# nka77/DAHiTra

Hardware: NVIDIA B200
Metric: image-pairs/sec (higher is better)
Workload: dtype x3 error-compensated f16 products (f16 main + scaled-remainder corrections; decoder: 3xTF32), fp32 accumulate

## Files before the change

### dahitra_b200/_lib.py

```python
from __future__ import annotations

import ctypes as C
import os
import subprocess
import threading

_HERE = os.path.dirname(os.path.abspath(__file__))
_CSRC = os.path.join(_HERE, "csrc")
LIB_PATH = os.path.join(_HERE, "libdahitra_b200.so")
SOURCES = ["conv_ffma.cu", "conv_tc.cu", "conv_tc2.cu", "conv_tc3.cu", "split.cu", "tokens.cu", "decoder.cu", "decoder_tc.cu", "stem_tc.cu", "classifier.cu", "train_decoder.cu", "train_tokens.cu", "prepare.cu", "aux.cu", "forward.cu"]
NVCC_FLAGS = ["-gencode", "arch=compute_100a,code=sm_100a", "-O3", "-lineinfo", "-std=c++17",
              "-Xcompiler", "-fPIC", "-shared"]

_lock = threading.Lock()
_lib = None


def _sources():
    return [os.path.join(_CSRC, s) for s in SOURCES if os.path.exists(os.path.join(_CSRC, s))]


STAMP_PATH = LIB_PATH + ".stamp"


def _deps():
    deps = _sources() + [os.path.join(_HERE, "..", "include", "dahitra_b200.h")]
    deps += [os.path.join(_CSRC, f) for f in sorted(os.listdir(_CSRC)) if f.endswith(".cuh")]
    return [d for d in deps if os.path.exists(d)]


def _source_hash() -> str:
    import hashlib
    h = hashlib.sha256(" ".join(NVCC_FLAGS + [os.environ.get("DAHITRA_DEBUG_BUILD", "0")]).encode())
    for d in _deps():
        h.update(os.path.basename(d).encode() + b"\0")
        with open(d, "rb") as f:
            h.update(f.read())
    return h.hexdigest()


def needs_build() -> bool:
    if not os.path.exists(LIB_PATH):
        return True
    if os.path.exists(STAMP_PATH):
        with open(STAMP_PATH) as f:
            return f.read().strip() != _source_hash()
    t = os.path.getmtime(LIB_PATH)
    if any(os.path.getmtime(d) > t for d in _deps()):
        return True
    _write_stamp()
    return False


def _write_stamp():
    try:
        with open(STAMP_PATH + ".tmp", "w") as f:
            f.write(_source_hash() + "\n")
        os.replace(STAMP_PATH + ".tmp", STAMP_PATH)
    except OSError:
        pass


def build(force: bool = False, verbose: bool = False) -> str:
    if not force and not needs_build():
        return LIB_PATH
    import tempfile
    from concurrent.futures import ThreadPoolExecutor
    nvcc = os.environ.get("NVCC", "nvcc")
    cflags = [f for f in NVCC_FLAGS if f != "-shared"]
    if os.environ.get("DAHITRA_DEBUG_BUILD") == "1":
        cflags.append("-DDH_MBAR_TIMEOUT")
    with tempfile.TemporaryDirectory(prefix="_build_", dir=_HERE) as tmp:
        def compile_one(src):
            obj = os.path.join(tmp, os.path.basename(src) + ".o")
            cmd = [nvcc] + cflags + ["-c", src, "-o", obj]
            if verbose:
                print(" ".join(cmd), flush=True)
            r = subprocess.run(cmd, capture_output=True, text=True)
            if r.returncode != 0:
                raise RuntimeError("nvcc failed on %s:\n%s%s" % (src, r.stdout, r.stderr))
            return obj
        with ThreadPoolExecutor(max_workers=min(8, os.cpu_count() or 1)) as ex:
            objs = list(ex.map(compile_one, _sources()))
        cmd = [nvcc] + NVCC_FLAGS + objs + ["-o", LIB_PATH + ".tmp"]
        if verbose:
            print(" ".join(cmd), flush=True)
        r = subprocess.run(cmd, capture_output=True, text=True)
        if r.returncode != 0:
            raise RuntimeError("nvcc link failed:\n" + r.stdout + r.stderr)
    os.replace(LIB_PATH + ".tmp", LIB_PATH)
    _write_stamp()
    return LIB_PATH


EXAMPLE_SRC = os.path.join(_HERE, "..", "examples", "dahitra_infer.c")
EXAMPLE_BIN = os.path.join(_HERE, "..", "examples", "bin", "dahitra_infer")


def build_example(force: bool = False, verbose: bool = False) -> str:
    src, out = os.path.abspath(EXAMPLE_SRC), os.path.abspath(EXAMPLE_BIN)
    deps = [src, LIB_PATH, os.path.join(_HERE, "..", "include", "dahitra_b200.h")]
    if not force and os.path.exists(out) and all(os.path.getmtime(d) <= os.path.getmtime(out) for d in deps):
        return out
    cuda = os.environ.get("CUDA_HOME", "/usr/local/cuda")
    os.makedirs(os.path.dirname(out), exist_ok=True)
    cmd = [os.environ.get("CC", "gcc"), "-std=c99", "-O2", "-Wall", "-Wextra", "-Werror", "-I", os.path.join(_HERE, "..", "include"),
           "-I", os.path.join(cuda, "include"), src, "-L", _HERE, "-ldahitra_b200", "-L", os.path.join(cuda, "lib64"),
           "-l:libcudart_static.a", "-ldl", "-lpthread", "-lrt", "-Wl,-rpath,$ORIGIN/../../dahitra_b200", "-o", out + ".tmp"]
    if verbose:
        print(" ".join(cmd), flush=True)
    r = subprocess.run(cmd, capture_output=True, text=True)
    if r.returncode != 0:
        raise RuntimeError("building examples/dahitra_infer.c failed:\n" + r.stdout + r.stderr)
    os.replace(out + ".tmp", out)
    return out


_P, _I, _LL, _SZ = C.c_void_p, C.c_int, C.c_longlong, C.c_size_t
SIGNATURES = {
    "dahitra_version": (_I, []),
    "dahitra_error_string": (C.c_char_p, [_I]),
    "dahitra_weight_slot_name": (C.c_char_p, [_I]),
    "dahitra_workspace_bytes": (_SZ, [_I, _I, _I, _I, _I, _I]),
    "dahitra_prepare_weights": (_LL, [_P, _I, _I, _I, _P, _LL, _P]),
    "dahitra_forward": (_I, [_P, _I, _P, _P, _LL, _P, _P, _P, _SZ, _I, _I, _I, _I, _I, _I, _P]),
    "dahitra_forward_profiled": (_I, [_P, _I, _P, _P, _LL, _P, _P, _P, _SZ, _I, _I, _I, _I, _I, _I, _P,
                                      _I, _P, _P, _P, _P]),
    "dahitra_conv2d": (_I, [_P, _P, _I, _I, _I, _I, _I, _I, _I, _I, _I, _I, _I, _P, _P, _P, _P, _I, _P, _I, _P]),
    "dahitra_conv2d_up2_tc": (_I, [_P, _I, _I, _I, _P, _P, _I, _P, _I, _P]),
    "dahitra_stem": (_I, [_P, _LL, _I, _I, _I, _P, _P, _P, _P]),
    "dahitra_stem_tc": (_I, [_P, _LL, _I, _I, _I, _P, _P, _P, _I, _P]),
    "dahitra_maxpool3x3s2": (_I, [_P, _I, _I, _I, _I, _P, _P]),
    "dahitra_squeeze_tokens": (_I, [_P, _I, _I, _I, _P, _P, _P, _P, _P]),
    "dahitra_token_encoder": (_I, [_P, _I, _I, _P, _I, _I, _P, _P]),
    "dahitra_decoder_tables": (_I, [_P, _I, _I, _I, _P, _I, _I, _P, _P]),
    "dahitra_pixel_decoder": (_I, [_P, _P, _P, _P, _I, _I, _I, _I, _I, _P, _I, _P, _P]),
    "dahitra_decoder_tables_tc": (_I, [_P, _I, _I, _I, _P, _I, _I, _P, _P]),
    "dahitra_pixel_decoder_tc": (_I, [_P, _P, _P, _P, _I, _I, _I, _I, _I, _P, _I, _I, _P, _P]),
    "dahitra_confusion_matrix": (_I, [_P, _P, _LL, _I, _P, _P]),
    "dahitra_prepare_input_u8": (_I, [_P, _I, _I, _I, _I, _I, _P, _P]),
    "dahitra_classifier": (_I, [_P, _I, _I, _I, _I, _P, _P, _P, _P, _P]),
    "dahitra_split_pack": (_I, [_P, _LL, _P, _P]),
    "dahitra_split_unpack": (_I, [_P, _LL, _P, _P]),
    "dahitra_maxpool3x3s2_split": (_I, [_P, _I, _I, _I, _I, _P, _P]),
    "dahitra_pixel_decoder_train_blocks": (_I, [_I]),
    "dahitra_pixel_decoder_train_fwd": (_I, [_P, _P, _P, _P, _I, _I, _I, _I, _I, _P]),
    "dahitra_pixel_decoder_train_bwd": (_I, [_P, _P, _P, _P, _P, _I, _I, _I, _I, _I, _P]),
    "dahitra_tokenizer_train_chunks": (_I, [_I]),
    "dahitra_tokenizer_train_fwd": (_I, [_P, _P, _P, _P, _P, _I, _I, _I, _P]),
    "dahitra_tokenizer_train_bwd": (_I, [_P, _P, _P, _P, _P, _P, _P, _I, _I, _I, _P]),
    "dahitra_conv2d_split": (_I, [_P, _P, _I, _I, _LL, _LL, _I, _I, _I, _I, _I, _I, _P, _P, _P, _I, _I, _P, _I, _I, _P, _P, _P]),
    "dahitra_maxpool3x3s2_h16": (_I, [_P, _I, _I, _I, _I, _P, _P]),
    "dahitra_classifier_h16": (_I, [_P, _I, _I, _I, _I, _P, _P, _P, _P, _P]),
}


class DhTensor(C.Structure):
    _fields_ = [("name", C.c_char_p), ("data", C.c_void_p), ("dtype", C.c_int), ("ndim", C.c_int), ("shape", C.c_longlong * 4)]


def load():
    global _lib
    with _lock:
        if _lib is None:
            if not os.path.exists(LIB_PATH):
                raise RuntimeError(
                    f"dahitra_b200: {LIB_PATH} is missing — run `python -c 'import __graft_entry__ as g; g.build()'` "
                    "(nvcc, sm_100a). There is no fallback path.")
            lib = C.CDLL(LIB_PATH)
            for name, (res, args) in SIGNATURES.items():
                fn = getattr(lib, name)
                fn.restype, fn.argtypes = res, args
            _lib = lib
        return _lib


def check(rc: int, what: str = "dahitra"):
    if rc != 0:
        msg = load().dahitra_error_string(rc)
        raise RuntimeError(f"{what} failed with code {rc}: {msg.decode() if msg else '?'}")
```

### dahitra_b200/csrc/common.cuh

```cuda
#pragma once
#include <cuda_runtime.h>
#include <stdint.h>
#include <stddef.h>
#include "../../include/dahitra_b200.h"

#ifndef __CUDA_ARCH_LIST__
#endif

#define DH_CHECK_LAUNCH()                                   \
  do {                                                      \
    cudaError_t e__ = cudaGetLastError();                   \
    if (e__ != cudaSuccess) return (int)e__;                \
  } while (0)

#define DH_REQUIRE(cond, code) \
  do {                         \
    if (!(cond)) return (code);\
  } while (0)

static inline bool dh_aligned16(const void* p) { return (reinterpret_cast<uintptr_t>(p) & 15u) == 0; }
static inline int dh_cdiv(int a, int b) { return (a + b - 1) / b; }

__device__ __forceinline__ float4 ldg4(const float* p) { return __ldg(reinterpret_cast<const float4*>(p)); }
__device__ __forceinline__ void st4(float* p, float4 v) { *reinterpret_cast<float4*>(p) = v; }

__device__ __forceinline__ float warp_sum(float v) {
#pragma unroll
  for (int o = 16; o > 0; o >>= 1) v += __shfl_xor_sync(0xffffffffu, v, o);
  return v;
}
__device__ __forceinline__ float warp_max(float v) {
#pragma unroll
  for (int o = 16; o > 0; o >>= 1) v = fmaxf(v, __shfl_xor_sync(0xffffffffu, v, o));
  return v;
}

__device__ __forceinline__ float gelu_erf(float x) { return 0.5f * x * (1.0f + erff(x * 0.70710678118654752440f)); }

struct ConvArgs {
  const float* in0; const float* in1; int C0, C1;
  int N, inH, inW, up;
  int KH, KW, stride, pad, Cout;
  const float* w;
  const float* wt;
  const float* bias; const float* res; int relu;
  float* out;
  int ps = 0;
  int flat = 0;
};
struct Conv3Args {
  const void* in0; const void* in1; int C0, C1;
  int N, inH, inW;
  long long in0_plane = 0, in1_plane = 0;
  long long res_plane = 0, out_plane = 0;
  int K, stride, Cout;
  const void* wt16;
  long long wt_plane_bytes;
  const float* bias; const void* res; int res_split;
  int relu;
  void* out; int out_split;
  int ps = 0;
  int tok = 0;
  const float* wtok = nullptr; float* partials = nullptr;
  int force_stream = 0;
  int cg = 0;
  int h16 = 0;
};
bool dh_conv_tc3_eligible(const Conv3Args& a);
int dh_launch_conv_tc3(const Conv3Args& a, cudaStream_t s);
int dh_conv_tc3_tok_chunks(int H, int W);
int dh_launch_split_pack(const float* in, size_t n, void* out, cudaStream_t s);
int dh_launch_split_unpack(const void* in, size_t n, float* out, cudaStream_t s);
int dh_launch_maxpool_split(const void* in, int N, int H, int W, int C, void* out, cudaStream_t s);
int dh_launch_maxpool_h16(const void* in, int N, int H, int W, int C, void* out, cudaStream_t s);
int dh_pdl_attr(cudaLaunchAttribute* at);
void dh_set_pdl(int on);
template <typename... KArgs, typename... Args>
static inline int dh_launch(void (*kern)(KArgs...), dim3 grid, dim3 block, size_t smem, cudaStream_t s, Args... args) {
  cudaLaunchConfig_t cfg = {};
  cfg.gridDim = grid; cfg.blockDim = block; cfg.dynamicSmemBytes = smem; cfg.stream = s;
  cudaLaunchAttribute at[1];
  cfg.attrs = at; cfg.numAttrs = dh_pdl_attr(at);
  const cudaError_t e = cudaLaunchKernelEx(&cfg, kern, KArgs(args)...);
  if (e != cudaSuccess) return (int)e;
  DH_CHECK_LAUNCH();
  return 0;
}
#ifdef __CUDACC__
__device__ __forceinline__ void dh_pdl_wait() { asm volatile("griddepcontrol.wait;" ::: "memory"); }
__device__ __forceinline__ void dh_pdl_launch_dependents() { asm volatile("griddepcontrol.launch_dependents;" ::: "memory"); }
#endif
int dh_launch_conv_ffma(const ConvArgs& a, cudaStream_t s);
bool dh_conv_tc_eligible(const ConvArgs& a);
int dh_launch_conv_tc(const ConvArgs& a, cudaStream_t s);
bool dh_conv_tc2_eligible(const ConvArgs& a);
int dh_launch_conv_tc2(const ConvArgs& a, int xm, int cg, cudaStream_t s);
int dh_launch_stem(const float* x, long long xbs, int N, int H, int W, const float* w, const float* b, float* out, cudaStream_t s);
int dh_launch_stem_tc(const float* x, long long xbs, int N, int H, int W, const float* wtc, const float* b, float* out, int x3,
                      cudaStream_t s, long long split_plane_pitch = 0, const float* x_second = nullptr);
int dh_launch_maxpool(const float* in, int N, int H, int W, int C, float* out, cudaStream_t s);
int dh_launch_classifier(const float* in, int N, int H, int W, int nc, const float* w, const float* b,
                         float* logits, unsigned char* amax, cudaStream_t s);
int dh_launch_classifier_tma(const float* in, int N, int H, int W, int nc, const float* w, const float* b,
                             float* logits, unsigned char* amax, cudaStream_t s);
int dh_launch_classifier_h16(const void* in, int N, int H, int W, int nc, const float* w, const float* b,
                             float* logits, unsigned char* amax, cudaStream_t s);
int dh_launch_squeeze_tokens(const float* feat, int N, int npix, int Cin, const float* wsq, const float* wtok,
                             float* xs, float* partials, cudaStream_t s);
int dh_launch_token_encoder(const float* partials, int B, int nchunk, const float* enc, int heads, int add_pos,
                            float* mem, cudaStream_t s);
int dh_launch_decoder_tables(const float* mem, int B, int first_call, int ncalls, const float* dec, int heads, int depth,
                             float* tables, cudaStream_t s);
int dh_launch_decoder_tables_tc(const float* mem, int B, int first_call, int ncalls, const float* dec, int heads, int depth,
                                float* tables, cudaStream_t s);
int dh_launch_pixel_decoder_tc(const float* x, const float* pos, const float* tables, const float* pack, int nimg, int h,
                               int w, int heads, int depth, const float* skip, int skip_up, int x3, float* out,
                               cudaStream_t s);
int dh_launch_pixel_decoder(const float* x, const float* pos, const float* tables, const float* dec,
                            int nimg, int h, int w, int heads, int depth, const float* skip, int skip_up, float* out,
                            cudaStream_t s);
```

### dahitra_b200/csrc/forward.cu

```cuda
#include "common.cuh"
#include <string.h>

namespace {

struct Level {
  int cin, heads, depth, h, w;
  size_t xs, xd, dx, out, part, mem, tab;
  int nchunk, nchunk3;
};

struct Plan {
  int B, H, W, nc, variant;
  size_t f2, p2, t4a, t4b, f4, t8a, t8b, t8c, f8, p8, t16a, t16b, t16c, f16;
  Level lv[3];
  size_t c4, c3, y20, o2, c2;
  size_t total_floats;
};

struct Bump {
  size_t off = 0;
  size_t take(size_t nfloats) {
    const size_t o = off;
    off += (nfloats + 63) & ~(size_t)63;
    return o;
  }
};

bool make_plan(Plan& p, int variant, int B, int H, int W, int nc, int flags) {
  if (B < 1 || H < 32 || W < 32 || (H % 32) || (W % 32) || nc < 1 || nc > 8) return false;
  if (variant != DH_VARIANT_LEVIR && variant != DH_VARIANT_XBD) return false;
  p.B = B; p.H = H; p.W = W; p.nc = nc; p.variant = variant;
  const size_t N2 = 2 * (size_t)B;
  const size_t s2 = (size_t)(H / 2) * (W / 2), s4 = s2 / 4, s8 = s4 / 4, s16 = s8 / 4;
  Bump b;
  p.f2 = b.take(N2 * s2 * 64);
  p.p2 = b.take(N2 * s4 * 64);
  p.t4a = b.take(N2 * s4 * 64); p.t4b = b.take(N2 * s4 * 64); p.f4 = b.take(N2 * s4 * 64);
  p.t8a = b.take(N2 * s8 * 128); p.t8b = b.take(N2 * s8 * 128); p.t8c = b.take(N2 * s8 * 128); p.f8 = b.take(N2 * s8 * 128);
  p.p8 = b.take(N2 * s16 * 128);
  p.t16a = b.take(N2 * s16 * 256); p.t16b = b.take(N2 * s16 * 256); p.t16c = b.take(N2 * s16 * 256); p.f16 = b.take(N2 * s16 * 256);
  const int cins[3] = {256, 128, 64}, heads[3] = {4, 4, 8}, depths[3] = {4, 4, 8}, div[3] = {16, 8, 4};
  for (int i = 0; i < 3; ++i) {
    Level& L = p.lv[i];
    L.cin = cins[i]; L.heads = heads[i]; L.depth = depths[i]; L.h = H / div[i]; L.w = W / div[i];
    const size_t n = (size_t)L.h * L.w;
    L.nchunk = (int)((n + 255) / 256);
    L.nchunk3 = dh_conv_tc3_tok_chunks(L.h, L.w);
    L.xs = b.take(N2 * n * 32);
    L.xd = b.take(N2 * n * 32);
    L.dx = b.take((size_t)B * n * 32);
    L.out = b.take((size_t)B * n * 32);
    L.part = b.take(N2 * (size_t)(L.nchunk3 > L.nchunk ? L.nchunk3 : L.nchunk) * 4 * 34);
    L.mem = b.take((size_t)B * 3 * 128);
    L.tab = b.take((size_t)3 * B * L.depth * (DH_TAB_FLOATS(L.heads) > DH_TABTC_FLOATS ? DH_TAB_FLOATS(L.heads) : DH_TABTC_FLOATS));
  }
  p.c4 = b.take((size_t)B * s4 * 32);
  const size_t n_c3 = (size_t)B * s2 * 32, n_y20 = (size_t)B * s2 * 128, n_c2 = (size_t)B * H * W * 32;
  const bool early_head = (flags & DH_FLAG_EARLY_HEAD) != 0;
  p.c3 = (p.t8c - p.t8a >= n_c3) ? p.t8a : b.take(n_c3);
  p.o2 = (p.p8 - p.t8c >= n_c3) ? p.t8c : b.take(n_c3);
  p.y20 = (!early_head && p.t8a - p.p2 >= n_y20) ? p.p2 : b.take(n_y20);
  p.c2 = (p.p2 - p.f2 >= n_c2) ? p.f2 : b.take(n_c2);
  p.total_floats = b.off;
  return true;
}

const char* kSlotNames[DH_W_COUNT] = {
  "DH_W_STEM_W", "DH_W_STEM_B",
  "DH_W_L1_0_C1_W", "DH_W_L1_0_C1_B", "DH_W_L1_0_C2_W", "DH_W_L1_0_C2_B",
  "DH_W_L1_1_C1_W", "DH_W_L1_1_C1_B", "DH_W_L1_1_C2_W", "DH_W_L1_1_C2_B",
  "DH_W_L2_0_C1_W", "DH_W_L2_0_C1_B", "DH_W_L2_0_C2_W", "DH_W_L2_0_C2_B", "DH_W_L2_0_DS_W", "DH_W_L2_0_DS_B",
  "DH_W_L2_1_C1_W", "DH_W_L2_1_C1_B", "DH_W_L2_1_C2_W", "DH_W_L2_1_C2_B",
  "DH_W_L3_0_C1_W", "DH_W_L3_0_C1_B", "DH_W_L3_0_C2_W", "DH_W_L3_0_C2_B", "DH_W_L3_0_DS_W", "DH_W_L3_0_DS_B",
  "DH_W_L3_1_C1_W", "DH_W_L3_1_C1_B", "DH_W_L3_1_C2_W", "DH_W_L3_1_C2_B",
  "DH_W_LV5_SQ", "DH_W_LV5_TOK", "DH_W_LV5_ENC", "DH_W_LV5_DEC", "DH_W_LV5_POS", "DH_W_LV5_DECODE",
  "DH_W_LV4_SQ", "DH_W_LV4_TOK", "DH_W_LV4_ENC", "DH_W_LV4_DEC", "DH_W_LV4_POS", "DH_W_LV4_DECODE",
  "DH_W_LV3_SQ", "DH_W_LV3_TOK", "DH_W_LV3_ENC", "DH_W_LV3_DEC", "DH_W_LV3_POS", "DH_W_LV3_DECODE",
  "DH_W_CL4_W", "DH_W_CL4_B", "DH_W_CL3_W", "DH_W_CL3_B", "DH_W_CL2_W", "DH_W_CL2_B",
  "DH_W_CL20A_W", "DH_W_CL20A_B", "DH_W_CL20B_W", "DH_W_CL20B_B", "DH_W_CLS_W", "DH_W_CLS_B",
  "DH_W_L1_0_C1_WT", "DH_W_L1_0_C2_WT", "DH_W_L1_1_C1_WT", "DH_W_L1_1_C2_WT",
  "DH_W_L2_0_C2_WT", "DH_W_L2_1_C1_WT", "DH_W_L2_1_C2_WT",
  "DH_W_L3_0_C1_WT", "DH_W_L3_0_C2_WT", "DH_W_L3_0_DS_WT", "DH_W_L3_1_C1_WT", "DH_W_L3_1_C2_WT",
  "DH_W_LV5_DECODE_WT", "DH_W_LV4_DECODE_WT", "DH_W_LV3_DECODE_WT", "DH_W_CL20A_WT", "DH_W_CL20B_WT",
  "DH_W_L2_0_C1_WT", "DH_W_L2_0_DS_WT",
  "DH_W_CL4_PSWT", "DH_W_CL4_PSB", "DH_W_CL3_PSWT", "DH_W_CL3_PSB", "DH_W_CL2_PSWT", "DH_W_CL2_PSB",
  "DH_W_LV5_DECTC", "DH_W_LV4_DECTC", "DH_W_LV3_DECTC", "DH_W_STEM_WTC",
  "DH_W_LV5_SQ_WT", "DH_W_LV4_SQ_WT", "DH_W_LV3_SQ_WT"};

int wt_slot_of(int wslot) {
  switch (wslot) {
    case DH_W_L1_0_C1_W: return DH_W_L1_0_C1_WT; case DH_W_L1_0_C2_W: return DH_W_L1_0_C2_WT;
    case DH_W_L1_1_C1_W: return DH_W_L1_1_C1_WT; case DH_W_L1_1_C2_W: return DH_W_L1_1_C2_WT;
    case DH_W_L2_0_C2_W: return DH_W_L2_0_C2_WT; case DH_W_L2_1_C1_W: return DH_W_L2_1_C1_WT;
    case DH_W_L2_1_C2_W: return DH_W_L2_1_C2_WT;
    case DH_W_L3_0_C1_W: return DH_W_L3_0_C1_WT; case DH_W_L3_0_C2_W: return DH_W_L3_0_C2_WT;
    case DH_W_L3_0_DS_W: return DH_W_L3_0_DS_WT; case DH_W_L3_1_C1_W: return DH_W_L3_1_C1_WT;
    case DH_W_L3_1_C2_W: return DH_W_L3_1_C2_WT;
    case DH_W_LV5_DECODE: return DH_W_LV5_DECODE_WT; case DH_W_LV4_DECODE: return DH_W_LV4_DECODE_WT;
    case DH_W_LV3_DECODE: return DH_W_LV3_DECODE_WT;
    case DH_W_CL20A_W: return DH_W_CL20A_WT; case DH_W_CL20B_W: return DH_W_CL20B_WT;
    case DH_W_L2_0_C1_W: return DH_W_L2_0_C1_WT; case DH_W_L2_0_DS_W: return DH_W_L2_0_DS_WT;
    default: return -1;
  }
}

}

extern "C" int dahitra_version(void) { return DAHITRA_ABI_VERSION; }

extern "C" const char* dahitra_error_string(int code) {
  switch (code) {
    case 0: return "ok";
    case DH_E_NULL: return "dahitra: required pointer is NULL";
    case DH_E_SHAPE: return "dahitra: unsupported shape";
    case DH_E_ALIGN: return "dahitra: pointer not 16-byte aligned";
    case DH_E_WORKSPACE: return "dahitra: workspace too small";
    case DH_E_VARIANT: return "dahitra: unknown variant or flags";
    case DH_E_WEIGHTS: return "dahitra: malformed weight table";
    default: return code > 0 ? cudaGetErrorString((cudaError_t)code) : "dahitra: unknown error";
  }
}

extern "C" const char* dahitra_weight_slot_name(int slot) {
  return (slot >= 0 && slot < DH_W_COUNT) ? kSlotNames[slot] : nullptr;
}

extern "C" size_t dahitra_workspace_bytes(int variant, int B, int H, int W, int output_nc, int flags) {
  Plan p;
  if (!make_plan(p, variant, B, H, W, output_nc, flags)) return 0;
  return p.total_floats * sizeof(float);
}

static int conv_dispatch(const ConvArgs& a, int flags, cudaStream_t s) {
  if (flags & DH_FLAG_CONV_TC) {
    const bool stride_ok = a.stride == 1 || (flags & DH_FLAG_TC_STRIDE2);
    if (stride_ok && !(flags & DH_FLAG_CONV_TC_V1) && dh_conv_tc2_eligible(a))
      return dh_launch_conv_tc2(a, (flags & DH_FLAG_TC_BF16) ? 3 : (flags & DH_FLAG_TC_3XTF32) ? ((flags & DH_FLAG_TC_MAIN_F16) ? ((flags & DH_FLAG_TC_FOLD) ? 6 : 4) : (flags & DH_FLAG_TC_X3_BF16) ? 2 : 1)
                                                            : ((flags & DH_FLAG_TC_MAIN_F16) ? 5 : 0),
                                (flags & DH_FLAG_CONV_TC_2CTA) ? 2 : 1, s);
    if (stride_ok && dh_conv_tc_eligible(a)) return dh_launch_conv_tc(a, s);
  }
  return dh_launch_conv_ffma(a, s);
}

extern "C" int dahitra_conv2d(const float* in0, const float* in1, int C0, int C1, int N, int inH, int inW, int up,
                              int KH, int KW, int stride, int pad, int Cout, const float* w, const float* wt,
                              const float* bias, const float* res, int relu, float* out, int flags, void* stream) {
  ConvArgs a{in0, in1, C0, C1, N, inH, inW, up, KH, KW, stride, pad, Cout, w, wt, bias, res, relu, out};
  return conv_dispatch(a, flags, (cudaStream_t)stream);
}
extern "C" int dahitra_conv2d_up2_tc(const float* in, int N, int inH, int inW, const float* pswt, const float* psb,
                                     int relu, float* out, int flags, void* stream) {
  ConvArgs a{in, nullptr, 32, 0, N, inH, inW, 1, 3, 3, 1, 1, 128, nullptr, pswt, psb, nullptr, relu, out};
  a.ps = 1;
  DH_REQUIRE(dh_conv_tc_eligible(a), DH_E_SHAPE);
  return conv_dispatch(a, flags | DH_FLAG_CONV_TC, (cudaStream_t)stream);
}
extern "C" int dahitra_stem(const float* x, long long xbs, int N, int H, int W, const float* w, const float* bias,
                            float* out, void* stream) {
  return dh_launch_stem(x, xbs, N, H, W, w, bias, out, (cudaStream_t)stream);
}
extern "C" int dahitra_stem_tc(const float* x, long long xbs, int N, int H, int W, const float* wtc, const float* bias,
                               float* out, int x3, void* stream) {
  return dh_launch_stem_tc(x, xbs, N, H, W, wtc, bias, out, x3, (cudaStream_t)stream);
}
extern "C" int dahitra_maxpool3x3s2(const float* in, int N, int H, int W, int C, float* out, void* stream) {
  return dh_launch_maxpool(in, N, H, W, C, out, (cudaStream_t)stream);
}
extern "C" int dahitra_squeeze_tokens(const float* feat, int N, int npix, int Cin, const float* w_sq, const float* w_tok,
                                      float* xs, float* partials, void* stream) {
  return dh_launch_squeeze_tokens(feat, N, npix, Cin, w_sq, w_tok, xs, partials, (cudaStream_t)stream);
}
extern "C" int dahitra_token_encoder(const float* partials, int B, int nchunk, const float* enc_pack, int heads,
                                     int add_pos, float* mem, void* stream) {
  return dh_launch_token_encoder(partials, B, nchunk, enc_pack, heads, add_pos, mem, (cudaStream_t)stream);
}
extern "C" int dahitra_decoder_tables(const float* mem, int B, int first_call, int ncalls, const float* dec_pack,
                                      int heads, int depth, float* tables, void* stream) {
  return dh_launch_decoder_tables(mem, B, first_call, ncalls, dec_pack, heads, depth, tables, (cudaStream_t)stream);
}
extern "C" int dahitra_pixel_decoder(const float* x, const float* pos, const float* tables, const float* dec_pack,
                                     int nimg, int h, int w, int heads, int depth, const float* skip, int skip_up,
                                     float* out, void* stream) {
  return dh_launch_pixel_decoder(x, pos, tables, dec_pack, nimg, h, w, heads, depth, skip, skip_up, out,
                                 (cudaStream_t)stream);
}
extern "C" int dahitra_decoder_tables_tc(const float* mem, int B, int first_call, int ncalls, const float* dec_pack,
                                         int heads, int depth, float* tables, void* stream) {
  return dh_launch_decoder_tables_tc(mem, B, first_call, ncalls, dec_pack, heads, depth, tables, (cudaStream_t)stream);
}
extern "C" int dahitra_pixel_decoder_tc(const float* x, const float* pos, const float* tables, const float* dectc_pack,
                                        int nimg, int h, int w, int heads, int depth, const float* skip, int skip_up,
                                        int x3, float* out, void* stream) {
  return dh_launch_pixel_decoder_tc(x, pos, tables, dectc_pack, nimg, h, w, heads, depth, skip, skip_up, x3, out,
                                    (cudaStream_t)stream);
}
extern "C" int dahitra_split_pack(const float* in, long long n, void* out, void* stream) {
  return dh_launch_split_pack(in, (size_t)n, out, (cudaStream_t)stream);
}
extern "C" int dahitra_split_unpack(const void* in, long long n, float* out, void* stream) {
  return dh_launch_split_unpack(in, (size_t)n, out, (cudaStream_t)stream);
}
extern "C" int dahitra_maxpool3x3s2_split(const void* in, int N, int H, int W, int C, void* out, void* stream) {
  return dh_launch_maxpool_split(in, N, H, W, C, out, (cudaStream_t)stream);
}
extern "C" int dahitra_conv2d_split(const void* in0, const void* in1, int C0, int C1, long long in0_plane, long long in1_plane,
                                    int N, int inH, int inW, int K, int stride, int Cout, const float* wt, const float* bias,
                                    const void* res, int res_split, int relu, void* out, int out_split, int mode,
                                    const float* w_tok, float* partials, void* stream) {
  DH_REQUIRE(wt, DH_E_NULL);
  const int h16 = (mode & 128) ? 1 : 0;
  const int sched = mode & ~(3 | 128);
  mode &= 3;
  DH_REQUIRE(mode <= 2 && !(sched & ~(16 | 32 | 64)), DH_E_VARIANT);
  Conv3Args a{};
  a.h16 = h16;
  a.cg = (sched & 32) ? 2 : ((sched & 16) ? 1 : 0);
  a.force_stream = (sched & 64) ? 1 : 0;
  a.in0 = in0; a.in1 = in1; a.C0 = C0; a.C1 = C1; a.N = N; a.inH = inH; a.inW = inW; a.in0_plane = in0_plane; a.in1_plane = in1_plane;
  a.K = K; a.stride = stride; a.Cout = Cout;
  const size_t plane = (size_t)Cout * K * K * (C0 + C1);
  a.wt16 = wt + 3 * plane; a.wt_plane_bytes = (long long)plane * 4;
  a.bias = bias; a.res = res; a.res_split = res_split; a.relu = relu; a.out = out; a.out_split = out_split;
  a.ps = mode == 1; a.tok = mode == 2; a.wtok = w_tok; a.partials = partials;
  return dh_launch_conv_tc3(a, (cudaStream_t)stream);
}
extern "C" int dahitra_classifier(const float* in, int N, int H, int W, int nc, const float* w, const float* bias,
                                  float* logits, unsigned char* argmax_u8, void* stream) {
  return dh_launch_classifier(in, N, H, W, nc, w, bias, logits, argmax_u8, (cudaStream_t)stream);
}
extern "C" int dahitra_maxpool3x3s2_h16(const void* in, int N, int H, int W, int C, void* out, void* stream) {
  return dh_launch_maxpool_h16(in, N, H, W, C, out, (cudaStream_t)stream);
}
extern "C" int dahitra_classifier_h16(const void* in, int N, int H, int W, int nc, const float* w, const float* bias,
                                      float* logits, unsigned char* argmax_u8, void* stream) {
  return dh_launch_classifier_h16(in, N, H, W, nc, w, bias, logits, argmax_u8, (cudaStream_t)stream);
}

namespace { thread_local int g_pdl = 0; }
void dh_set_pdl(int on) { g_pdl = on; }
int dh_pdl_attr(cudaLaunchAttribute* at) {
  if (!g_pdl) return 0;
  at[0].id = cudaLaunchAttributeProgrammaticStreamSerialization;
  at[0].val.programmaticStreamSerializationAllowed = 1;
  return 1;
}

namespace {
constexpr int PROF_MAX = 160;
struct ProfRec { const char* name; double flops, bytes; };
struct Profiler {
  bool on = false, created = false;
  int n = 0;
  cudaEvent_t ev[PROF_MAX + 1];
  ProfRec rec[PROF_MAX];
};
thread_local Profiler g_prof;

inline void prof_mark(cudaStream_t s, const char* name, double flops, double bytes) {
  if (!g_prof.on || g_prof.n >= PROF_MAX) return;
  g_prof.rec[g_prof.n] = {name, flops, bytes};
  ++g_prof.n;
  cudaEventRecord(g_prof.ev[g_prof.n], s);
}
}

namespace {
struct AuxStreams {
  bool ok = false;
  cudaStream_t st[2], low;
  cudaEvent_t fork, join[2], fork_low, join_low;
};
AuxStreams* aux_streams() {
  thread_local AuxStreams per_dev[16];
  int dev = 0;
  if (cudaGetDevice(&dev) != cudaSuccess || dev < 0 || dev >= 16) return nullptr;
  AuxStreams& a = per_dev[dev];
  if (!a.ok) {
    bool good = cudaEventCreateWithFlags(&a.fork, cudaEventDisableTiming) == cudaSuccess;
    for (int i = 0; i < 2 && good; ++i)
      good = cudaStreamCreateWithFlags(&a.st[i], cudaStreamNonBlocking) == cudaSuccess &&
             cudaEventCreateWithFlags(&a.join[i], cudaEventDisableTiming) == cudaSuccess;
    if (good) {
      int lo = 0, hi = 0;
      cudaDeviceGetStreamPriorityRange(&lo, &hi);
      good = cudaStreamCreateWithPriority(&a.low, cudaStreamNonBlocking, lo) == cudaSuccess &&
             cudaEventCreateWithFlags(&a.fork_low, cudaEventDisableTiming) == cudaSuccess &&
             cudaEventCreateWithFlags(&a.join_low, cudaEventDisableTiming) == cudaSuccess;
    }
    if (!good) { cudaGetLastError(); return nullptr; }
    a.ok = true;
  }
  return &a;
}
}

#define DH_STEP(name, fl, by, expr)        \
  do {                                     \
    const int rc__ = (expr);               \
    if (rc__ != 0) return rc__;            \
    prof_mark(s, name, (fl), (by));        \
  } while (0)

namespace {
int forward_split(const Plan& p, const void* const* weights, const float* x1, const float* x2, long long x_batch_stride,
                  float* logits, unsigned char* argmax_u8, float* ws, int variant, int B, int H, int W, int output_nc, int flags,
                  cudaStream_t s_main) {
  cudaStream_t s = s_main;
  auto Wt = [&](int slot) { return (const float*)weights[slot]; };
  const int N2 = 2 * B;
  const int h2 = H / 2, w2 = W / 2, h4 = H / 4, w4 = W / 4, h8 = H / 8, w8 = W / 8, h16 = H / 16, w16 = W / 16;
  const bool one = (flags & DH_FLAG_ACT_H16) != 0;
  const double eb = one ? 2.0 : 4.0;
  auto conv3 = [&](const char* name, const float* in0, const float* in1, int C0, int C1, long long in_plane, int N, int inH, int inW,
                   int K, int stride, int Cout, int wts, int bslot, const float* res, int res_split, int relu, float* out,
                   int out_split, int ps) -> int {
    Conv3Args a{};
    a.in0 = in0; a.in1 = in1; a.C0 = C0; a.C1 = C1; a.N = N; a.inH = inH; a.inW = inW; a.in0_plane = in_plane; a.in1_plane = in_plane;
    a.K = K; a.stride = stride; a.Cout = Cout;
    const size_t plane = (size_t)Cout * K * K * (C0 + C1);
    a.wt16 = Wt(wts) + 3 * plane; a.wt_plane_bytes = (long long)plane * 4;
    a.bias = bslot >= 0 ? Wt(bslot) : nullptr; a.res = res; a.res_split = one ? 1 : res_split; a.relu = relu; a.out = out;
    a.out_split = one ? 1 : out_split;
    a.ps = ps; a.h16 = one;
    const int rc = dh_launch_conv_tc3(a, s);
    if (rc != 0) return rc;
    const double OH = (double)inH / stride, OW = (double)inW / stride, Cin = C0 + C1;
    const double cout_alg = ps ? 32.0 : Cout, up = ps ? 2.0 : 1.0;
    const double fl = 2.0 * N * OH * up * OW * up * cout_alg * K * K * Cin;
    const double by = eb * ((double)N * inH * inW * Cin + (double)N * OH * up * OW * up * cout_alg * (res ? 2 : 1) + (double)K * K * Cin * cout_alg);
    prof_mark(s, name, fl, by);
    return 0;
  };
#define DH_CONV3(...)                     \
  do {                                    \
    const int rc__ = conv3(__VA_ARGS__);  \
    if (rc__ != 0) return rc__;           \
  } while (0)

  auto H16 = [](float* p) { return reinterpret_cast<uint16_t*>(p); };
  float* F2 = ws + p.f2;
  const size_t f2_half = (size_t)B * h2 * w2 * 64;
  const long long f2_plane = (long long)N2 * h2 * w2 * 64;
  float* F2post = reinterpret_cast<float*>(H16(F2) + f2_half);
  const double stem_fl = 2.0 * B * h2 * w2 * 64 * 147;
  const double stem_by = one ? B * (4.0 * 3 * H * W + 2.0 * h2 * w2 * 64) : 4.0 * B * ((double)3 * H * W + (double)h2 * w2 * 64);
  const int stem_mode = one ? 3 | 512 : ((flags & DH_FLAG_TC_3XTF32) ? 2 : 3) | 256;
  DH_STEP("stem", 2.0 * stem_fl, 2.0 * stem_by,
          dh_launch_stem_tc(x1, x_batch_stride, B, H, W, Wt(DH_W_STEM_WTC), Wt(DH_W_STEM_B), F2, stem_mode, s, f2_plane, x2));
  float* P2 = ws + p.p2;
  auto maxpool = [&](const float* in, int hh, int ww, int C, float* out) {
    return one ? dh_launch_maxpool_h16(in, N2, hh, ww, C, out, s) : dh_launch_maxpool_split(in, N2, hh, ww, C, out, s);
  };
  DH_STEP("maxpool_2", 0.0, eb * N2 * 64 * ((double)h2 * w2 + (double)h4 * w4), maxpool(F2, h2, w2, 64, P2));
  float *T4a = ws + p.t4a, *T4b = ws + p.t4b, *F4 = ws + p.f4;
  DH_CONV3("layer1.0.conv1", P2, nullptr, 64, 0, 0, N2, h4, w4, 3, 1, 64, DH_W_L1_0_C1_WT, DH_W_L1_0_C1_B, nullptr, 0, 1, T4a, 1, 0);
  DH_CONV3("layer1.0.conv2", T4a, nullptr, 64, 0, 0, N2, h4, w4, 3, 1, 64, DH_W_L1_0_C2_WT, DH_W_L1_0_C2_B, P2, 1, 1, T4b, 1, 0);
  DH_CONV3("layer1.1.conv1", T4b, nullptr, 64, 0, 0, N2, h4, w4, 3, 1, 64, DH_W_L1_1_C1_WT, DH_W_L1_1_C1_B, nullptr, 0, 1, T4a, 1, 0);
  DH_CONV3("layer1.1.conv2", T4a, nullptr, 64, 0, 0, N2, h4, w4, 3, 1, 64, DH_W_L1_1_C2_WT, DH_W_L1_1_C2_B, T4b, 1, 1, F4, 1, 0);
  float *T8a = ws + p.t8a, *T8b = ws + p.t8b, *T8c = ws + p.t8c, *F8 = ws + p.f8;
  DH_CONV3("layer2.0.conv1", F4, nullptr, 64, 0, 0, N2, h4, w4, 3, 2, 128, DH_W_L2_0_C1_WT, DH_W_L2_0_C1_B, nullptr, 0, 1, T8a, 1, 0);
  DH_CONV3("layer2.0.down", F4, nullptr, 64, 0, 0, N2, h4, w4, 1, 2, 128, DH_W_L2_0_DS_WT, DH_W_L2_0_DS_B, nullptr, 0, 0, T8b, 1, 0);
  DH_CONV3("layer2.0.conv2", T8a, nullptr, 128, 0, 0, N2, h8, w8, 3, 1, 128, DH_W_L2_0_C2_WT, DH_W_L2_0_C2_B, T8b, 1, 1, T8c, 1, 0);
  DH_CONV3("layer2.1.conv1", T8c, nullptr, 128, 0, 0, N2, h8, w8, 3, 1, 128, DH_W_L2_1_C1_WT, DH_W_L2_1_C1_B, nullptr, 0, 1, T8a, 1, 0);
  DH_CONV3("layer2.1.conv2", T8a, nullptr, 128, 0, 0, N2, h8, w8, 3, 1, 128, DH_W_L2_1_C2_WT, DH_W_L2_1_C2_B, T8c, 1, 1, F8, 1, 0);
  float* P8 = ws + p.p8;
  DH_STEP("maxpool_8", 0.0, eb * N2 * 128 * ((double)h8 * w8 + (double)h16 * w16), maxpool(F8, h8, w8, 128, P8));
  float *T16a = ws + p.t16a, *T16b = ws + p.t16b, *T16c = ws + p.t16c, *F16 = ws + p.f16;
  DH_CONV3("layer3.0.conv1", P8, nullptr, 128, 0, 0, N2, h16, w16, 3, 1, 256, DH_W_L3_0_C1_WT, DH_W_L3_0_C1_B, nullptr, 0, 1, T16a, 1, 0);
  DH_CONV3("layer3.0.down", P8, nullptr, 128, 0, 0, N2, h16, w16, 1, 1, 256, DH_W_L3_0_DS_WT, DH_W_L3_0_DS_B, nullptr, 0, 0, T16b, 1, 0);
  DH_CONV3("layer3.0.conv2", T16a, nullptr, 256, 0, 0, N2, h16, w16, 3, 1, 256, DH_W_L3_0_C2_WT, DH_W_L3_0_C2_B, T16b, 1, 1, T16c, 1, 0);
  DH_CONV3("layer3.1.conv1", T16c, nullptr, 256, 0, 0, N2, h16, w16, 3, 1, 256, DH_W_L3_1_C1_WT, DH_W_L3_1_C1_B, nullptr, 0, 1, T16a, 1, 0);
  DH_CONV3("layer3.1.conv2", T16a, nullptr, 256, 0, 0, N2, h16, w16, 3, 1, 256, DH_W_L3_1_C2_WT, DH_W_L3_1_C2_B, T16c, 1, 1, F16, 1, 0);

  float* feats[3] = {F16, F8, F4};
  const int base[3] = {DH_W_LV5_SQ, DH_W_LV4_SQ, DH_W_LV3_SQ};
  static const char* const nm[3][7] = {
      {"squeeze_tok_5", "token_enc_5", "dec_tables_5", "decoder_5_x12", "conv_decode_5", "decoder_5_diff", "conv_layer4"},
      {"squeeze_tok_4", "token_enc_4", "dec_tables_4", "decoder_4_x12", "conv_decode_4", "decoder_4_diff", "conv_layer4"},
      {"squeeze_tok_3", "token_enc_3", "dec_tables_3", "decoder_3_x12", "conv_decode_3", "decoder_3_diff", "conv_layer4"}};
  float* C4 = ws + p.c4;
  const int x3 = (flags & DH_FLAG_DEC_TC_X3) ? 1 : 0;
  auto dec_bytes_px = [&](const float* pos) { return one ? 32.0 * (2 + 2 + (pos ? 4 : 0)) : 4.0 * 32 * (pos ? 3 : 2); };
  auto level_pre = [&](int i) -> int {
    const Level& L = p.lv[i];
    const int npix = L.h * L.w;
    const float *wtok = Wt(base[i] + 1), *enc = Wt(base[i] + 2), *dec = Wt(base[i] + 3), *pos = Wt(base[i] + 4);
    float *XS = ws + L.xs, *XD = ws + L.xd, *DX = ws + L.dx, *PART = ws + L.part, *MEM = ws + L.mem, *TAB = ws + L.tab;
    const double inner = 64.0 * L.heads;
    const double dec_fl_px = L.depth * 2.0 * (32 * inner + 4 * inner + 4 * inner + inner * 32 + 2 * 32 * 32);
    const double dec_by_px = dec_bytes_px(pos);
    const bool levir = variant == DH_VARIANT_LEVIR;
    {
      Conv3Args a{};
      a.in0 = feats[i]; a.C0 = L.cin; a.N = N2; a.inH = L.h; a.inW = L.w; a.K = 1; a.stride = 1; a.Cout = 32;
      const size_t plane = (size_t)32 * L.cin;
      a.wt16 = Wt(DH_W_LV5_SQ_WT + i) + 3 * plane; a.wt_plane_bytes = (long long)plane * 4;
      a.out = XS; a.out_split = (levir && !one) ? 0 : 1; a.tok = 1; a.wtok = wtok; a.partials = PART; a.h16 = one;
      DH_STEP(nm[i][0], 2.0 * N2 * npix * 32 * (L.cin + 4 + 4), eb * N2 * npix * (L.cin + 32.0), dh_launch_conv_tc3(a, s));
    }
    const int add_tok_pos = levir ? 1 : (i == 0 ? 1 : 0);
    DH_STEP(nm[i][1], 0.0, 4.0 * N2 * L.nchunk3 * 136.0, dh_launch_token_encoder(PART, B, L.nchunk3, enc, L.heads, add_tok_pos, MEM, s));
    const size_t half = (size_t)B * npix * 32;
    const long long plane2 = (long long)N2 * npix * 32;
    const float* dectc = Wt(DH_W_LV5_DECTC + i);
    if (levir) {
      DH_STEP(nm[i][2], 0.0, 4.0 * 3 * B * L.depth * (double)DH_TABTC_FLOATS, dh_launch_decoder_tables_tc(MEM, B, 0, 3, dec, L.heads, L.depth, TAB, s));
      DH_STEP(nm[i][3], dec_fl_px * N2 * npix, dec_by_px * N2 * npix,
              dh_launch_pixel_decoder_tc(XS, pos, TAB, dectc, N2, L.h, L.w, L.heads, L.depth, nullptr, 1, x3 | (one ? 512 : 256), XD, s));
      DH_CONV3(nm[i][4], XD, reinterpret_cast<float*>(H16(XD) + half), 32, 32, plane2, B, L.h, L.w, 3, 1, 32, DH_W_LV5_DECODE_WT + i, -1,
               nullptr, 0, 0, DX, 0, 0);
    } else {
      DH_STEP(nm[i][2], 0.0, 4.0 * B * L.depth * (double)DH_TABTC_FLOATS, dh_launch_decoder_tables_tc(MEM, B, 2, 1, dec, L.heads, L.depth, TAB, s));
      DH_CONV3(nm[i][4], XS, reinterpret_cast<float*>(H16(XS) + half), 32, 32, plane2, B, L.h, L.w, 3, 1, 32, DH_W_LV5_DECODE_WT + i, -1,
               nullptr, 0, 0, DX, 0, 0);
    }
    return 0;
  };
  auto level_post = [&](int i) -> int {
    const Level& L = p.lv[i];
    const int npix = L.h * L.w;
    const float* pos = Wt(base[i] + 4);
    float *DX = ws + L.dx, *OUT = ws + L.out, *TAB = ws + L.tab;
    const float* skip = (i == 0) ? nullptr : (i == 1 ? ws + p.lv[0].out : C4);
    const int skip_up = (i == 1) ? 2 : 1;
    const double inner = 64.0 * L.heads;
    const double dec_fl_px = L.depth * 2.0 * (32 * inner + 4 * inner + 4 * inner + inner * 32 + 2 * 32 * 32);
    const double dec_by_px = dec_bytes_px(pos);
    const float* dectc = Wt(DH_W_LV5_DECTC + i);
    const float* tab2 = (variant == DH_VARIANT_LEVIR) ? TAB + (size_t)2 * B * L.depth * DH_TABTC_FLOATS : TAB;
    const int out_split = one ? 512 : (i == 0 ? 0 : 256);
    DH_STEP(nm[i][5], dec_fl_px * B * npix, (dec_by_px + (skip ? 32.0 * eb / (skip_up * skip_up) : 0.0)) * B * npix,
            dh_launch_pixel_decoder_tc(DX, pos, tab2, dectc, B, L.h, L.w, L.heads, L.depth, skip, skip_up, x3 | out_split, OUT, s));
    if (i == 1)
      DH_CONV3(nm[i][6], OUT, nullptr, 32, 0, 0, B, L.h, L.w, 3, 1, 128, DH_W_CL4_PSWT, DH_W_CL4_PSB, nullptr, 0, 1, C4, 0, 1);
    return 0;
  };
  AuxStreams* aux = (g_prof.on || (flags & DH_FLAG_SERIAL)) ? nullptr : aux_streams();
  if (aux) {
    if (cudaEventRecord(aux->fork, s_main) != cudaSuccess) return (int)cudaGetLastError();
    for (int i = 1; i <= 2; ++i) {
      s = aux->st[i - 1];
      if (cudaStreamWaitEvent(s, aux->fork, 0) != cudaSuccess) return (int)cudaGetLastError();
      const int rc = level_pre(i);
      if (rc == 0 && cudaEventRecord(aux->join[i - 1], s) != cudaSuccess) { s = s_main; return (int)cudaGetLastError(); }
      s = s_main;
      if (rc != 0) return rc;
    }
  }
  for (int i = 0; i < 3; ++i) {
    int rc = 0;
    if (i == 0 || !aux) rc = level_pre(i);
    else if (cudaStreamWaitEvent(s_main, aux->join[i - 1], 0) != cudaSuccess) rc = (int)cudaGetLastError();
    if (rc == 0) rc = level_post(i);
    if (rc != 0) return rc;
  }
  float *C3 = ws + p.c3, *Y20 = ws + p.y20, *O2 = ws + p.o2, *C2 = ws + p.c2;
  float* OUT3 = ws + p.lv[2].out;
  DH_CONV3("conv_layer3", OUT3, nullptr, 32, 0, 0, B, h4, w4, 3, 1, 128, DH_W_CL3_PSWT, DH_W_CL3_PSB, nullptr, 0, 1, C3, 0, 1);
  DH_CONV3("conv_layer2_0.0", F2, F2post, 64, 64, f2_plane, B, h2, w2, 3, 1, 128, DH_W_CL20A_WT, DH_W_CL20A_B, nullptr, 0, 1, Y20, 1, 0);
  DH_CONV3("conv_layer2_0.3", Y20, nullptr, 128, 0, 0, B, h2, w2, 3, 1, 32, DH_W_CL20B_WT, DH_W_CL20B_B, C3, 0, 0, O2, 1, 0);
  DH_CONV3("conv_layer2", O2, nullptr, 32, 0, 0, B, h2, w2, 3, 1, 128, DH_W_CL2_PSWT, DH_W_CL2_PSB, nullptr, 0, 1, C2, 0, 1);
  DH_STEP("classifier", 2.0 * B * H * W * 9 * 32 * output_nc,
          (one ? B * H * W * (2.0 * 32 + 4.0 * output_nc) : 4.0 * B * H * W * (32.0 + output_nc)) + (argmax_u8 ? (double)B * H * W : 0.0),
          one ? dh_launch_classifier_h16(C2, B, H, W, output_nc, Wt(DH_W_CLS_W), Wt(DH_W_CLS_B), logits, argmax_u8, s)
              : dh_launch_classifier(C2, B, H, W, output_nc, Wt(DH_W_CLS_W), Wt(DH_W_CLS_B), logits, argmax_u8, s));
  return 0;
}
}


extern "C" int dahitra_forward(const void* const* weights, int n_weights, const float* x1, const float* x2,
                               long long x_batch_stride, float* logits, unsigned char* argmax_u8, void* workspace,
                               size_t workspace_bytes, int variant, int B, int H, int W, int output_nc, int flags,
                               void* stream) {
  DH_REQUIRE(weights && x1 && x2 && logits && workspace, DH_E_NULL);
  DH_REQUIRE(n_weights == DH_W_COUNT, DH_E_WEIGHTS);
  Plan p;
  DH_REQUIRE(variant == DH_VARIANT_LEVIR || variant == DH_VARIANT_XBD, DH_E_VARIANT);
  if (flags & DH_FLAG_ACT_H16) {
    constexpr int need = DH_FLAG_CONV_TC | DH_FLAG_TC_MAIN_F16 | DH_FLAG_TC_STRIDE2 | DH_FLAG_STEM_TC | DH_FLAG_DEC_TC;
    DH_REQUIRE((flags & need) == need &&
               !(flags & (DH_FLAG_ACT_SPLIT | DH_FLAG_TC_3XTF32 | DH_FLAG_TC_BF16 | DH_FLAG_CONV_TC_V1)), DH_E_VARIANT);
  }
  DH_REQUIRE(make_plan(p, variant, B, H, W, output_nc, flags), DH_E_SHAPE);
  DH_REQUIRE(workspace_bytes >= p.total_floats * sizeof(float), DH_E_WORKSPACE);
  DH_REQUIRE(dh_aligned16(workspace), DH_E_ALIGN);
  for (int i = 0; i < DH_W_COUNT; ++i) {
    const bool optional = (i == DH_W_LV5_POS || i == DH_W_LV4_POS || i == DH_W_LV3_POS);
    DH_REQUIRE(weights[i] || optional, DH_E_WEIGHTS);
    DH_REQUIRE(dh_aligned16(weights[i]), DH_E_ALIGN);
  }
  const cudaStream_t s_main = (cudaStream_t)stream;
  cudaStream_t s = s_main;
  float* ws = (float*)workspace;
  dh_set_pdl((flags & DH_FLAG_PDL) ? 1 : 0);
  if (flags & DH_FLAG_ACT_SPLIT) {
    constexpr int need = DH_FLAG_CONV_TC | DH_FLAG_TC_MAIN_F16 | DH_FLAG_TC_STRIDE2 | DH_FLAG_STEM_TC | DH_FLAG_DEC_TC;
    DH_REQUIRE((flags & need) == need && !(flags & (DH_FLAG_TC_BF16 | DH_FLAG_CONV_TC_V1)), DH_E_VARIANT);
    return forward_split(p, weights, x1, x2, x_batch_stride, logits, argmax_u8, ws, variant, B, H, W, output_nc, flags, s_main);
  }
  if (flags & DH_FLAG_ACT_H16)
    return forward_split(p, weights, x1, x2, x_batch_stride, logits, argmax_u8, ws, variant, B, H, W, output_nc, flags, s_main);
  auto Wt = [&](int slot) { return (const float*)weights[slot]; };
  const int N2 = 2 * B;
  const int h2 = H / 2, w2 = W / 2, h4 = H / 4, w4 = W / 4, h8 = H / 8, w8 = W / 8, h16 = H / 16, w16 = W / 16;

  int conv_flat = 0;
  auto conv = [&](const char* name, const float* in0, const float* in1, int C0, int C1, int N, int inH, int inW, int up,
                  int K, int stride, int Cout, int wslot, int bslot, const float* res, int relu, float* out) -> int {
    const int wts = wt_slot_of(wslot);
    ConvArgs a{in0, in1, C0, C1, N, inH, inW, up, K, K, stride, K / 2, Cout, Wt(wslot), wts >= 0 ? Wt(wts) : nullptr,
               bslot >= 0 ? Wt(bslot) : nullptr, res, relu, out};
    const int psw = (wslot == DH_W_CL4_W) ? DH_W_CL4_PSWT : (wslot == DH_W_CL3_W) ? DH_W_CL3_PSWT
                  : (wslot == DH_W_CL2_W) ? DH_W_CL2_PSWT : -1;
    a.flat = conv_flat;
    if (up == 2 && psw >= 0 && (flags & DH_FLAG_CONV_TC)) {
      a.up = 1; a.Cout = 128; a.w = nullptr; a.wt = Wt(psw); a.bias = Wt(psw + 1); a.ps = 1;
    }
    const int rc = conv_dispatch(a, flags, s);
    if (rc != 0) return rc;
    const double OH = (double)(inH * up) / stride, OW = (double)(inW * up) / stride, Cin = C0 + C1;
    const double fl = 2.0 * N * OH * OW * Cout * K * K * Cin;
    const double by = 4.0 * ((double)N * inH * inW * Cin + (double)N * OH * OW * Cout * (res ? 2 : 1) + (double)K * K * Cin * Cout);
    prof_mark(s, name, fl, by);
    return 0;
  };
#define DH_CONV(...)                     \
  do {                                   \
    const int rc__ = conv(__VA_ARGS__);  \
    if (rc__ != 0) return rc__;          \
  } while (0)

  float* F2 = ws + p.f2;
  const double stem_fl = 2.0 * B * h2 * w2 * 64 * 147, stem_by = 4.0 * B * ((double)3 * H * W + (double)h2 * w2 * 64);
  const int stem_mode = !(flags & DH_FLAG_TC_3XTF32)
                            ? ((flags & (DH_FLAG_TC_MAIN_F16 | DH_FLAG_TC_BF16)) ? 3 : 0)
                            : ((flags & DH_FLAG_TC_FOLD) && (flags & DH_FLAG_TC_MAIN_F16) && (flags & DH_FLAG_TC_X3_BF16)) ? 2 : 1;
  auto stem = [&](const float* xin, float* o) -> int {
    return (flags & DH_FLAG_STEM_TC) ? dh_launch_stem_tc(xin, x_batch_stride, B, H, W, Wt(DH_W_STEM_WTC), Wt(DH_W_STEM_B), o,
                                                         stem_mode, s)
                                     : dh_launch_stem(xin, x_batch_stride, B, H, W, Wt(DH_W_STEM_W), Wt(DH_W_STEM_B), o, s);
  };
  DH_STEP("stem_pre", stem_fl, stem_by, stem(x1, F2));
  DH_STEP("stem_post", stem_fl, stem_by, stem(x2, F2 + (size_t)B * h2 * w2 * 64));
  AuxStreams* aux_head = (!g_prof.on && !(flags & DH_FLAG_SERIAL) && (flags & DH_FLAG_EARLY_HEAD) && (flags & DH_FLAG_CONV_TC))
                             ? aux_streams() : nullptr;
  float* Y20 = ws + p.y20;
  if (aux_head) {
    if (cudaEventRecord(aux_head->fork_low, s_main) != cudaSuccess ||
        cudaStreamWaitEvent(aux_head->low, aux_head->fork_low, 0) != cudaSuccess) return (int)cudaGetLastError();
    s = aux_head->low; conv_flat = 1;
    const int rc = conv("conv_layer2_0.0", F2, F2 + (size_t)B * h2 * w2 * 64, 64, 64, B, h2, w2, 1, 3, 1, 128, DH_W_CL20A_W, DH_W_CL20A_B,
                        nullptr, 1, Y20);
    conv_flat = 0;
    const bool ok = rc == 0 && cudaEventRecord(aux_head->join_low, s) == cudaSuccess;
    s = s_main;
    if (!ok) return rc != 0 ? rc : (int)cudaGetLastError();
  }
  float* P2 = ws + p.p2;
  DH_STEP("maxpool_2", 0.0, 4.0 * N2 * 64 * ((double)h2 * w2 + (double)h4 * w4), dh_launch_maxpool(F2, N2, h2, w2, 64, P2, s));
  float *T4a = ws + p.t4a, *T4b = ws + p.t4b, *F4 = ws + p.f4;
  DH_CONV("layer1.0.conv1", P2, nullptr, 64, 0, N2, h4, w4, 1, 3, 1, 64, DH_W_L1_0_C1_W, DH_W_L1_0_C1_B, nullptr, 1, T4a);
  DH_CONV("layer1.0.conv2", T4a, nullptr, 64, 0, N2, h4, w4, 1, 3, 1, 64, DH_W_L1_0_C2_W, DH_W_L1_0_C2_B, P2, 1, T4b);
  DH_CONV("layer1.1.conv1", T4b, nullptr, 64, 0, N2, h4, w4, 1, 3, 1, 64, DH_W_L1_1_C1_W, DH_W_L1_1_C1_B, nullptr, 1, T4a);
  DH_CONV("layer1.1.conv2", T4a, nullptr, 64, 0, N2, h4, w4, 1, 3, 1, 64, DH_W_L1_1_C2_W, DH_W_L1_1_C2_B, T4b, 1, F4);
  float *T8a = ws + p.t8a, *T8b = ws + p.t8b, *T8c = ws + p.t8c, *F8 = ws + p.f8;
  DH_CONV("layer2.0.conv1", F4, nullptr, 64, 0, N2, h4, w4, 1, 3, 2, 128, DH_W_L2_0_C1_W, DH_W_L2_0_C1_B, nullptr, 1, T8a);
  DH_CONV("layer2.0.down", F4, nullptr, 64, 0, N2, h4, w4, 1, 1, 2, 128, DH_W_L2_0_DS_W, DH_W_L2_0_DS_B, nullptr, 0, T8b);
  DH_CONV("layer2.0.conv2", T8a, nullptr, 128, 0, N2, h8, w8, 1, 3, 1, 128, DH_W_L2_0_C2_W, DH_W_L2_0_C2_B, T8b, 1, T8c);
  DH_CONV("layer2.1.conv1", T8c, nullptr, 128, 0, N2, h8, w8, 1, 3, 1, 128, DH_W_L2_1_C1_W, DH_W_L2_1_C1_B, nullptr, 1, T8a);
  DH_CONV("layer2.1.conv2", T8a, nullptr, 128, 0, N2, h8, w8, 1, 3, 1, 128, DH_W_L2_1_C2_W, DH_W_L2_1_C2_B, T8c, 1, F8);
  float* P8 = ws + p.p8;
  DH_STEP("maxpool_8", 0.0, 4.0 * N2 * 128 * ((double)h8 * w8 + (double)h16 * w16), dh_launch_maxpool(F8, N2, h8, w8, 128, P8, s));
  float *T16a = ws + p.t16a, *T16b = ws + p.t16b, *T16c = ws + p.t16c, *F16 = ws + p.f16;
  DH_CONV("layer3.0.conv1", P8, nullptr, 128, 0, N2, h16, w16, 1, 3, 1, 256, DH_W_L3_0_C1_W, DH_W_L3_0_C1_B, nullptr, 1, T16a);
  DH_CONV("layer3.0.down", P8, nullptr, 128, 0, N2, h16, w16, 1, 1, 1, 256, DH_W_L3_0_DS_W, DH_W_L3_0_DS_B, nullptr, 0, T16b);
  DH_CONV("layer3.0.conv2", T16a, nullptr, 256, 0, N2, h16, w16, 1, 3, 1, 256, DH_W_L3_0_C2_W, DH_W_L3_0_C2_B, T16b, 1, T16c);
  DH_CONV("layer3.1.conv1", T16c, nullptr, 256, 0, N2, h16, w16, 1, 3, 1, 256, DH_W_L3_1_C1_W, DH_W_L3_1_C1_B, nullptr, 1, T16a);
  DH_CONV("layer3.1.conv2", T16a, nullptr, 256, 0, N2, h16, w16, 1, 3, 1, 256, DH_W_L3_1_C2_W, DH_W_L3_1_C2_B, T16c, 1, F16);

  const float* feats[3] = {F16, F8, F4};
  const int base[3] = {DH_W_LV5_SQ, DH_W_LV4_SQ, DH_W_LV3_SQ};
  static const char* const nm[3][7] = {
      {"squeeze_tok_5", "token_enc_5", "dec_tables_5", "decoder_5_x12", "conv_decode_5", "decoder_5_diff", "conv_layer4"},
      {"squeeze_tok_4", "token_enc_4", "dec_tables_4", "decoder_4_x12", "conv_decode_4", "decoder_4_diff", "conv_layer4"},
      {"squeeze_tok_3", "token_enc_3", "dec_tables_3", "decoder_3_x12", "conv_decode_3", "decoder_3_diff", "conv_layer4"}};
  float* C4 = ws + p.c4;
  auto level_pre = [&](int i) -> int {
    const Level& L = p.lv[i];
    const int npix = L.h * L.w;
    const float *wsq = Wt(base[i] + 0), *wtok = Wt(base[i] + 1), *enc = Wt(base[i] + 2), *dec = Wt(base[i] + 3),
                *pos = Wt(base[i] + 4);
    float *XS = ws + L.xs, *XD = ws + L.xd, *DX = ws + L.dx, *PART = ws + L.part, *MEM = ws + L.mem, *TAB = ws + L.tab;
    const double inner = 64.0 * L.heads;
    const double dec_fl_px = L.depth * 2.0 * (32 * inner + 4 * inner + 4 * inner + inner * 32 + 2 * 32 * 32);
    const double dec_by_px = 4.0 * 32 * (pos ? 3 : 2);
    DH_STEP(nm[i][0], 2.0 * N2 * npix * 32 * (L.cin + 4 + 4), 4.0 * N2 * npix * (L.cin + 32.0),
            dh_launch_squeeze_tokens(feats[i], N2, npix, L.cin, wsq, wtok, XS, PART, s));
    const int add_tok_pos = (variant == DH_VARIANT_LEVIR) ? 1 : (i == 0 ? 1 : 0);
    DH_STEP(nm[i][1], 0.0, 4.0 * N2 * L.nchunk * 136.0, dh_launch_token_encoder(PART, B, L.nchunk, enc, L.heads, add_tok_pos, MEM, s));
    const size_t half = (size_t)B * npix * 32;
    const bool dtc = (flags & DH_FLAG_DEC_TC) != 0;
    const float* dectc = Wt(DH_W_LV5_DECTC + i);
    const size_t tabf = dtc ? (size_t)DH_TABTC_FLOATS : (size_t)DH_TAB_FLOATS(L.heads);
    auto tables = [&](int first, int ncalls) -> int {
      return dtc ? dh_launch_decoder_tables_tc(MEM, B, first, ncalls, dec, L.heads, L.depth, TAB, s)
                 : dh_launch_decoder_tables(MEM, B, first, ncalls, dec, L.heads, L.depth, TAB, s);
    };
    if (variant == DH_VARIANT_LEVIR) {
      DH_STEP(nm[i][2], 0.0, 4.0 * 3 * B * L.depth * tabf, tables(0, 3));
      DH_STEP(nm[i][3], dec_fl_px * N2 * npix, dec_by_px * N2 * npix,
              (dtc ? dh_launch_pixel_decoder_tc(XS, pos, TAB, dectc, N2, L.h, L.w, L.heads, L.depth, nullptr, 1,
                                                (flags & DH_FLAG_DEC_TC_X3) ? 1 : 0, XD, s)
                   : dh_launch_pixel_decoder(XS, pos, TAB, dec, N2, L.h, L.w, L.heads, L.depth, nullptr, 1, XD, s)));
      DH_CONV(nm[i][4], XD, XD + half, 32, 32, B, L.h, L.w, 1, 3, 1, 32, base[i] + 5, -1, nullptr, 0, DX);
    } else {
      DH_STEP(nm[i][2], 0.0, 4.0 * B * L.depth * tabf, tables(2, 1));
      DH_CONV(nm[i][4], XS, XS + half, 32, 32, B, L.h, L.w, 1, 3, 1, 32, base[i] + 5, -1, nullptr, 0, DX);
    }
    return 0;
  };
  auto level_post = [&](int i) -> int {
    const Level& L = p.lv[i];
    const int npix = L.h * L.w;
    const float *dec = Wt(base[i] + 3), *pos = Wt(base[i] + 4);
    float *DX = ws + L.dx, *OUT = ws + L.out, *TAB = ws + L.tab;
    const float* skip = (i == 0) ? nullptr : (i == 1 ? ws + p.lv[0].out : C4);
    const int skip_up = (i == 1) ? 2 : 1;
    const double inner = 64.0 * L.heads;
    const double dec_fl_px = L.depth * 2.0 * (32 * inner + 4 * inner + 4 * inner + inner * 32 + 2 * 32 * 32);
    const double dec_by_px = 4.0 * 32 * (pos ? 3 : 2);
    const bool dtc = (flags & DH_FLAG_DEC_TC) != 0;
    const float* dectc = Wt(DH_W_LV5_DECTC + i);
    const size_t tabf = dtc ? (size_t)DH_TABTC_FLOATS : (size_t)DH_TAB_FLOATS(L.heads);
    const float* tab2 = (variant == DH_VARIANT_LEVIR) ? TAB + (size_t)2 * B * L.depth * tabf : TAB;
    DH_STEP(nm[i][5], dec_fl_px * B * npix, (dec_by_px + (skip ? 128.0 / (skip_up * skip_up) : 0.0)) * B * npix,
            (dtc ? dh_launch_pixel_decoder_tc(DX, pos, tab2, dectc, B, L.h, L.w, L.heads, L.depth, skip, skip_up,
                                              (flags & DH_FLAG_DEC_TC_X3) ? 1 : 0, OUT, s)
                 : dh_launch_pixel_decoder(DX, pos, tab2, dec, B, L.h, L.w, L.heads, L.depth, skip, skip_up, OUT, s)));
    if (i == 1)
      DH_CONV(nm[i][6], OUT, nullptr, 32, 0, B, L.h, L.w, 2, 3, 1, 32, DH_W_CL4_W, DH_W_CL4_B, nullptr, 1, C4);
    return 0;
  };
  AuxStreams* aux = (g_prof.on || (flags & DH_FLAG_SERIAL)) ? nullptr : aux_streams();
  if (aux) {
    if (cudaEventRecord(aux->fork, s_main) != cudaSuccess) return (int)cudaGetLastError();
    for (int i = 1; i <= 2; ++i) {
      s = aux->st[i - 1];
      if (cudaStreamWaitEvent(s, aux->fork, 0) != cudaSuccess) return (int)cudaGetLastError();
      const int rc = level_pre(i);
      if (rc == 0 && cudaEventRecord(aux->join[i - 1], s) != cudaSuccess) { s = s_main; return (int)cudaGetLastError(); }
      s = s_main;
      if (rc != 0) return rc;
    }
  }
  for (int i = 0; i < 3; ++i) {
    int rc = 0;
    if (i == 0 || !aux) rc = level_pre(i);
    else if (cudaStreamWaitEvent(s_main, aux->join[i - 1], 0) != cudaSuccess) rc = (int)cudaGetLastError();
    if (rc == 0) rc = level_post(i);
    if (rc != 0) return rc;
  }
  float *C3 = ws + p.c3, *O2 = ws + p.o2, *C2 = ws + p.c2;
  const float* OUT3 = ws + p.lv[2].out;
  DH_CONV("conv_layer3", OUT3, nullptr, 32, 0, B, h4, w4, 2, 3, 1, 32, DH_W_CL3_W, DH_W_CL3_B, nullptr, 1, C3);
  const float* A128 = F2;
  const float* B128 = F2 + (size_t)B * h2 * w2 * 64;
  if (aux_head) {
    if (cudaStreamWaitEvent(s_main, aux_head->join_low, 0) != cudaSuccess) return (int)cudaGetLastError();
  } else {
    DH_CONV("conv_layer2_0.0", A128, B128, 64, 64, B, h2, w2, 1, 3, 1, 128, DH_W_CL20A_W, DH_W_CL20A_B, nullptr, 1, Y20);
  }
  DH_CONV("conv_layer2_0.3", Y20, nullptr, 128, 0, B, h2, w2, 1, 3, 1, 32, DH_W_CL20B_W, DH_W_CL20B_B, C3, 0, O2);
  DH_CONV("conv_layer2", O2, nullptr, 32, 0, B, h2, w2, 2, 3, 1, 32, DH_W_CL2_W, DH_W_CL2_B, nullptr, 1, C2);
  DH_STEP("classifier", 2.0 * B * H * W * 9 * 32 * output_nc, 4.0 * B * H * W * (32.0 + output_nc) + (argmax_u8 ? (double)B * H * W : 0.0),
          dh_launch_classifier(C2, B, H, W, output_nc, Wt(DH_W_CLS_W), Wt(DH_W_CLS_B), logits, argmax_u8, s));
  return 0;
}

extern "C" int dahitra_forward_profiled(const void* const* weights, int n_weights, const float* x1, const float* x2,
                                        long long x_batch_stride, float* logits, unsigned char* argmax_u8,
                                        void* workspace, size_t workspace_bytes, int variant, int B, int H, int W,
                                        int output_nc, int flags, void* stream, int cap, float* ms, double* flops,
                                        double* bytes, const char** names) {
  DH_REQUIRE(ms && flops && bytes && names && cap > 0, DH_E_NULL);
  cudaStream_t s = (cudaStream_t)stream;
  if (!g_prof.created) {
    for (int i = 0; i <= PROF_MAX; ++i)
      if (cudaEventCreate(&g_prof.ev[i]) != cudaSuccess) return -(int)cudaGetLastError() - 1000;
    g_prof.created = true;
  }
  g_prof.n = 0;
  g_prof.on = true;
  cudaEventRecord(g_prof.ev[0], s);
  const int rc = dahitra_forward(weights, n_weights, x1, x2, x_batch_stride, logits, argmax_u8, workspace, workspace_bytes,
                                 variant, B, H, W, output_nc, flags, stream);
  g_prof.on = false;
  if (rc != 0) return rc > 0 ? -rc - 1000 : rc;
  const cudaError_t e = cudaStreamSynchronize(s);
  if (e != cudaSuccess) return -(int)e - 1000;
  const int n = g_prof.n < cap ? g_prof.n : cap;
  for (int i = 0; i < n; ++i) {
    cudaEventElapsedTime(&ms[i], g_prof.ev[i], g_prof.ev[i + 1]);
    flops[i] = g_prof.rec[i].flops;
    bytes[i] = g_prof.rec[i].bytes;
    names[i] = g_prof.rec[i].name;
  }
  return n;
}
```

### dahitra_b200/csrc/stem_tc.cu

```cuda
#include "tc_common.cuh"

using namespace dhtc;

namespace {
constexpr int SK_TH = 8, SK_TW = 16;
constexpr int SK_HR = 2 * SK_TH + 5;
constexpr int SK_HCP = 40;
constexpr int SK_PLANE = SK_HR * SK_HCP;
constexpr int SK_KSTEPS = 6;
constexpr int SK_GROUPS = 21;
constexpr uint32_t SK_A_BYTES = 128 * 128;
constexpr uint32_t SK_B_BYTES = SK_KSTEPS * 64 * 128;
constexpr uint32_t SK_HALO_BYTES = 3 * SK_PLANE * 4;
constexpr uint32_t SK_HALO_STRIDE = 10112;
constexpr uint32_t SK_IDESC = umma_idesc_tf32(128, 64);
constexpr int SK_THREADS = 14 * 32;

template <bool X3> struct SkCfg {
  static constexpr uint32_t NA = X3 ? 4 : 2;
  static constexpr uint32_t NB = X3 ? 2 : 1;
  static constexpr uint32_t OFF_B = NA * SK_A_BYTES;
  static constexpr uint32_t OFF_H = OFF_B + NB * SK_B_BYTES;
  static constexpr uint32_t OFF_E = OFF_H + 2 * SK_HALO_STRIDE;
  static constexpr uint32_t SMEM = OFF_E + 4 * 4096 + 1024;
};

__device__ __forceinline__ float sk_tf32(float v) { return tf32_round(v); }

struct SkTile { int n, oy0, ox0; };
__device__ __forceinline__ SkTile sk_tile(int t, int tilesX, int tilesY) {
  SkTile r;
  r.ox0 = (t % tilesX) * SK_TW; t /= tilesX;
  r.oy0 = (t % tilesY) * SK_TH;
  r.n = t / tilesY;
  return r;
}

__device__ __forceinline__ void sk_halo_producer(const CUtensorMap* tmX, uint32_t halo_addr, uint64_t* halo_full, uint64_t* halo_free,
                                                 int tilesX, int tilesY, int ntiles, const CUtensorMap* tmX2 = nullptr, int nfirst = 1 << 30) {
  int it = 0;
  for (int tile = blockIdx.x; tile < ntiles; tile += gridDim.x, ++it) {
    const int hb = it & 1;
    if (it >= 2) mbar_wait(smem_u32(&halo_free[hb]), (uint32_t)(((it >> 1) - 1) & 1));
    const SkTile tl = sk_tile(tile, tilesX, tilesY);
    const uint32_t bar = smem_u32(&halo_full[hb]);
    mbar_expect_tx(bar, SK_HALO_BYTES);
    const bool second = tl.n >= nfirst;
    tma_load_4d(halo_addr + (uint32_t)hb * SK_HALO_STRIDE, second ? tmX2 : tmX, bar, 2 * tl.ox0 - 4, 2 * tl.oy0 - 3, 0, second ? tl.n - nfirst : tl.n);
  }
}

__device__ __forceinline__ void sk_store_slice(const float (&v)[32], float* stage, int lane, int q, int j, const SkTile& t,
                                               int OH, int OW, const float* __restrict__ bias, float* __restrict__ out,
                                               long long split_plane = 0) {
  const int c4 = lane & 3, r4 = lane >> 2;
#pragma unroll
  for (int k4 = 0; k4 < 8; ++k4)
    *reinterpret_cast<float4*>(stage + lane * 32 + ((k4 ^ (lane & 7)) << 2)) = make_float4(v[k4 * 4], v[k4 * 4 + 1], v[k4 * 4 + 2], v[k4 * 4 + 3]);
  __syncwarp();
  const float4 b0 = ldg4(bias + j * 32 + c4 * 8), b1 = ldg4(bias + j * 32 + c4 * 8 + 4);
#pragma unroll
  for (int g = 0; g < 4; ++g) {
    const int r = g * 8 + r4, mm = q * 32 + r;
    const int oy = t.oy0 + mm / SK_TW, ox = t.ox0 + mm % SK_TW;
    const float4 o0 = *reinterpret_cast<const float4*>(stage + r * 32 + (((2 * c4) ^ (r & 7)) << 2));
    const float4 o1 = *reinterpret_cast<const float4*>(stage + r * 32 + (((2 * c4 + 1) ^ (r & 7)) << 2));
    if (oy < OH && ox < OW) {
      const float4 r0 = make_float4(fmaxf(o0.x + b0.x, 0.f), fmaxf(o0.y + b0.y, 0.f), fmaxf(o0.z + b0.z, 0.f), fmaxf(o0.w + b0.w, 0.f));
      const float4 r1 = make_float4(fmaxf(o1.x + b1.x, 0.f), fmaxf(o1.y + b1.y, 0.f), fmaxf(o1.z + b1.z, 0.f), fmaxf(o1.w + b1.w, 0.f));
      const size_t off = ((size_t)(t.n * OH + oy) * OW + ox) * 64 + j * 32 + c4 * 8;
      if (split_plane < 0) {
        uint4 hi;
        hi.x = pack_f16x2_sat(r0.x, r0.y); hi.y = pack_f16x2_sat(r0.z, r0.w); hi.z = pack_f16x2_sat(r1.x, r1.y); hi.w = pack_f16x2_sat(r1.z, r1.w);
        *reinterpret_cast<uint4*>(reinterpret_cast<uint16_t*>(out) + off) = hi;
      } else if (split_plane) {
        uint4 hi, lo;
        hi.x = pack_f16x2_sat(r0.x, r0.y); hi.y = pack_f16x2_sat(r0.z, r0.w); hi.z = pack_f16x2_sat(r1.x, r1.y); hi.w = pack_f16x2_sat(r1.z, r1.w);
        lo.x = pack_f16x2_sat((r0.x - f16_lo(hi.x)) * 2048.f, (r0.y - f16_hi(hi.x)) * 2048.f);
        lo.y = pack_f16x2_sat((r0.z - f16_lo(hi.y)) * 2048.f, (r0.w - f16_hi(hi.y)) * 2048.f);
        lo.z = pack_f16x2_sat((r1.x - f16_lo(hi.z)) * 2048.f, (r1.y - f16_hi(hi.z)) * 2048.f);
        lo.w = pack_f16x2_sat((r1.z - f16_lo(hi.w)) * 2048.f, (r1.w - f16_hi(hi.w)) * 2048.f);
        uint16_t* o16 = reinterpret_cast<uint16_t*>(out);
        *reinterpret_cast<uint4*>(o16 + off) = hi;
        *reinterpret_cast<uint4*>(o16 + off + (size_t)split_plane) = lo;
      } else {
        st4(out + off, r0); st4(out + off + 4, r1);
      }
    }
  }
  __syncwarp();
}

template <bool X3>
__global__ void __launch_bounds__(SK_THREADS, 1)
stem_tc_kernel(const __grid_constant__ CUtensorMap tmX, int OH, int OW, int tilesX, int tilesY, int ntiles,
               const float* __restrict__ wtc, const float* __restrict__ bias, float* __restrict__ out) {
  using Cfg = SkCfg<X3>;
  extern __shared__ uint8_t sk_raw[];
  __shared__ __align__(8) uint64_t w_bar, a_full[2], a_free[2], acc_full[2], acc_empty[2], halo_full[2], halo_free[2];
  __shared__ uint32_t tmem_slot;
  const int tid = threadIdx.x, warp = tid >> 5;
  const uint32_t base = (smem_u32(sk_raw) + 1023u) & ~1023u;
  uint8_t* bp = sk_raw + (base - smem_u32(sk_raw));
  constexpr uint32_t A_LO = 2 * SK_A_BYTES;
  const uint32_t b_addr = base + Cfg::OFF_B;

  if (tid == 0) {
    mbar_init(smem_u32(&w_bar), 1);
    for (int i = 0; i < 2; ++i) {
      mbar_init(smem_u32(&a_full[i]), 128);
      mbar_init(smem_u32(&a_free[i]), 1);
      mbar_init(smem_u32(&acc_full[i]), 1);
      mbar_init(smem_u32(&acc_empty[i]), 128);
      mbar_init(smem_u32(&halo_full[i]), 1);
      mbar_init(smem_u32(&halo_free[i]), 256);
    }
    mbar_fence_init();
  }
  if (warp == 0) tmem_alloc(smem_u32(&tmem_slot), 128);
  tc_fence_before();
  __syncthreads();
  tc_fence_after();
  const uint32_t tmem_base = tmem_slot;

  if (warp < 8) {
    const int wg = warp >> 2, t = tid & 127;
    const int py = t / SK_TW, px = t % SK_TW;
    const int pbase = (2 * py) * SK_HCP + 2 * px;
    const int swz = t & 7;
    int it = 0, use = 0;
    for (int tile = blockIdx.x; tile < ntiles; tile += gridDim.x, ++it) {
      const int hb = it & 1;
      mbar_wait(smem_u32(&halo_full[hb]), (uint32_t)((it >> 1) & 1));
      const float* halo = reinterpret_cast<const float*>(bp + Cfg::OFF_H + (size_t)hb * SK_HALO_STRIDE) + pbase;
      float* at = reinterpret_cast<float*>(bp + (size_t)wg * SK_A_BYTES) + t * 32;
#pragma unroll 1
      for (int kt = wg; kt < SK_KSTEPS; kt += 2, ++use) {
        if (use >= 1) mbar_wait(smem_u32(&a_free[wg]), (uint32_t)((use - 1) & 1));
#pragma unroll
        for (int j = 0; j < 4; ++j) {
          const int g = kt * 4 + j;
          float v[8];
          if (g < SK_GROUPS) {
            const float2* src = reinterpret_cast<const float2*>(halo + (g / 7) * SK_PLANE + (g % 7) * SK_HCP);
#pragma unroll
            for (int q = 0; q < 4; ++q) { const float2 f = src[q]; v[2 * q] = f.x; v[2 * q + 1] = f.y; }
          } else {
#pragma unroll
            for (int q = 0; q < 8; ++q) v[q] = 0.f;
          }
#pragma unroll
          for (int c = 0; c < 2; ++c) {
            const int o = ((2 * j + c) ^ swz) << 2;
            const float h0 = sk_tf32(v[c * 4]), h1 = sk_tf32(v[c * 4 + 1]), h2 = sk_tf32(v[c * 4 + 2]), h3 = sk_tf32(v[c * 4 + 3]);
            *reinterpret_cast<float4*>(at + o) = make_float4(h0, h1, h2, h3);
            if (X3) *reinterpret_cast<float4*>(at + A_LO / 4 + o) = make_float4(sk_tf32(v[c * 4] - h0), sk_tf32(v[c * 4 + 1] - h1),
                                                                              sk_tf32(v[c * 4 + 2] - h2), sk_tf32(v[c * 4 + 3] - h3));
          }
        }
        fence_async_smem();
        mbar_arrive_local(smem_u32(&a_full[wg]));
      }
      mbar_arrive_local(smem_u32(&halo_free[hb]));
    }
  } else if (warp < 12) {
    const int q = warp & 3, lane = tid & 31;
    float* stage = reinterpret_cast<float*>(bp + Cfg::OFF_E + (size_t)q * 4096);
    int it = 0;
    for (int tile = blockIdx.x; tile < ntiles; tile += gridDim.x, ++it) {
      const SkTile t = sk_tile(tile, tilesX, tilesY);
      const int ab = it & 1;
      mbar_wait(smem_u32(&acc_full[ab]), (uint32_t)((it >> 1) & 1));
      tc_fence_after();
      const uint32_t tm = tmem_base + ((uint32_t)(q * 32) << 16) + (uint32_t)ab * 64;
#pragma unroll 1
      for (int j = 0; j < 2; ++j) {
        uint32_t u[32];
        float v[32];
        tmem_ld32(tm + (uint32_t)(j * 32), u);
        if (j == 1) {
          tc_fence_before();
          mbar_arrive_local(smem_u32(&acc_empty[ab]));
        }
#pragma unroll
        for (int i = 0; i < 32; ++i) v[i] = __uint_as_float(u[i]);
        sk_store_slice(v, stage, lane, q, j, t, OH, OW, bias, out);
      }
    }
  } else if (warp == 13) {
    if ((tid & 31) == 0) sk_halo_producer(&tmX, base + Cfg::OFF_H, halo_full, halo_free, tilesX, tilesY, ntiles);
  } else if ((tid & 31) == 0) {
    mbar_expect_tx(smem_u32(&w_bar), Cfg::NB * SK_B_BYTES);
    bulk_load_1d(b_addr, wtc, SK_B_BYTES, smem_u32(&w_bar));
    if (X3) bulk_load_1d(b_addr + SK_B_BYTES, wtc + SK_B_BYTES / 4, SK_B_BYTES, smem_u32(&w_bar));
    mbar_wait(smem_u32(&w_bar), 0);
    int it = 0;
    uint32_t full_phase[2] = {0, 0};
    for (int tile = blockIdx.x; tile < ntiles; tile += gridDim.x, ++it) {
      const int ab = it & 1;
      mbar_wait(smem_u32(&acc_empty[ab]), (uint32_t)(((it >> 1) & 1) ^ 1));
      tc_fence_after();
      const uint32_t d = tmem_base + (uint32_t)ab * 64;
#pragma unroll
      for (int kt = 0; kt < SK_KSTEPS; ++kt) {
        const int buf = kt & 1;
        mbar_wait(smem_u32(&a_full[buf]), full_phase[buf]);
        full_phase[buf] ^= 1u;
        tc_fence_after();
        const uint32_t a_addr = base + (uint32_t)buf * SK_A_BYTES;
        const uint64_t ad = umma_desc_sw128(a_addr), bd = umma_desc_sw128(b_addr + (uint32_t)kt * 64 * 128);
#pragma unroll
        for (int k = 0; k < 4; ++k) umma_tf32(d, ad + (uint64_t)(2 * k), bd + (uint64_t)(2 * k), SK_IDESC, (kt | k) ? 1u : 0u);
        if (X3) {
          const uint64_t al = umma_desc_sw128(a_addr + A_LO), bl = umma_desc_sw128(b_addr + SK_B_BYTES + (uint32_t)kt * 64 * 128);
#pragma unroll
          for (int k = 0; k < 4; ++k) umma_tf32(d, al + (uint64_t)(2 * k), bd + (uint64_t)(2 * k), SK_IDESC, 1u);
#pragma unroll
          for (int k = 0; k < 4; ++k) umma_tf32(d, ad + (uint64_t)(2 * k), bl + (uint64_t)(2 * k), SK_IDESC, 1u);
        }
        umma_commit(smem_u32(&a_free[buf]));
      }
      umma_commit(smem_u32(&acc_full[ab]));
    }
  }
  tc_fence_before();
  __syncthreads();
  if (warp == 0) {
    tc_fence_after();
    tmem_dealloc(tmem_base, 128);
  }
}
constexpr int SF_KSTEPS = 3;
constexpr int SF_NBUF = 3;
constexpr uint32_t SF_A_BUF = 2 * SK_A_BYTES;
constexpr uint32_t SF_BM_STEP = 128 * 128;
constexpr uint32_t SF_BC_STEP = 64 * 128;
constexpr uint32_t SF_BM_BYTES = SF_KSTEPS * SF_BM_STEP, SF_BC_BYTES = SF_KSTEPS * SF_BC_STEP;
constexpr uint32_t SF_OFF_B = SF_NBUF * SF_A_BUF;
constexpr uint32_t SF_OFF_H = SF_OFF_B + SF_BM_BYTES + SF_BC_BYTES;
constexpr uint32_t SF_OFF_E = SF_OFF_H + 2 * SK_HALO_STRIDE;
constexpr uint32_t SF_SMEM = SF_OFF_E + 4 * 4096 + 1024;
constexpr uint32_t SF_IDESC_MAIN = umma_idesc_f16(128, 128), SF_IDESC_CORR = umma_idesc_bf16(128, 64), SF_IDESC_ONE = umma_idesc_f16(128, 64);
constexpr size_t SF_IMAGE_OFFSET_FLOATS = 2 * (SK_B_BYTES / 4);

template <bool FOLD>
__global__ void __launch_bounds__(SK_THREADS, 1)
stem_f16_kernel(const __grid_constant__ CUtensorMap tmX, const __grid_constant__ CUtensorMap tmX2, int nfirst, int OH, int OW, int tilesX,
                int tilesY, int ntiles, const float* __restrict__ wtc, const float* __restrict__ bias, float* __restrict__ out,
                long long split_plane) {
  extern __shared__ uint8_t sk_raw[];
  __shared__ __align__(8) uint64_t w_bar, a_full[SF_NBUF], a_free[SF_NBUF], acc_full[2], acc_empty[2], halo_full[2], halo_free[2];
  __shared__ uint32_t tmem_slot;
  const int tid = threadIdx.x, warp = tid >> 5;
  const uint32_t base = (smem_u32(sk_raw) + 1023u) & ~1023u;
  uint8_t* bp = sk_raw + (base - smem_u32(sk_raw));
  const uint32_t b_addr = base + SF_OFF_B;

  if (tid == 0) {
    mbar_init(smem_u32(&w_bar), 1);
    for (int i = 0; i < SF_NBUF; ++i) {
      mbar_init(smem_u32(&a_full[i]), 128);
      mbar_init(smem_u32(&a_free[i]), 1);
    }
    for (int i = 0; i < 2; ++i) {
      mbar_init(smem_u32(&acc_full[i]), 1);
      mbar_init(smem_u32(&acc_empty[i]), 128);
      mbar_init(smem_u32(&halo_full[i]), 1);
      mbar_init(smem_u32(&halo_free[i]), 256);
    }
    mbar_fence_init();
  }
  if (warp == 0) tmem_alloc(smem_u32(&tmem_slot), 256);
  tc_fence_before();
  __syncthreads();
  tc_fence_after();
  const uint32_t tmem_base = tmem_slot;
  dh_pdl_wait();
  dh_pdl_launch_dependents();

  if (warp < 8) {
    const int wg = warp >> 2, t = tid & 127;
    const int py = t / SK_TW, px = t % SK_TW;
    const int pbase = (2 * py) * SK_HCP + 2 * px;
    const int swz = t & 7;
    int it = 0, c = wg, buf = wg, use = 0;
    for (int tile = blockIdx.x; tile < ntiles; tile += gridDim.x, ++it) {
      const int hb = it & 1;
      mbar_wait(smem_u32(&halo_full[hb]), (uint32_t)((it >> 1) & 1));
      const float* halo = reinterpret_cast<const float*>(bp + SF_OFF_H + (size_t)hb * SK_HALO_STRIDE) + pbase;
#pragma unroll 1
      for (; c < SF_KSTEPS * (it + 1); c += 2) {
        const int kt = c - SF_KSTEPS * it;
        if (use >= 1) mbar_wait(smem_u32(&a_free[buf]), (uint32_t)((use - 1) & 1));
        uint8_t* row = bp + (size_t)buf * SF_A_BUF + t * 128;
        const int ng = kt == 2 ? 6 : 8;
#pragma unroll
        for (int j = 0; j < 8; ++j) {
          if (j < ng) {
            const int g = kt * 8 + j;
            uint4 hi = make_uint4(0u, 0u, 0u, 0u), lo = hi;
            if (g < SK_GROUPS) {
              const float2* src = reinterpret_cast<const float2*>(halo + (g / 7) * SK_PLANE + (g % 7) * SK_HCP);
              const float2 f0 = src[0], f1 = src[1], f2 = src[2], f3 = src[3];
              hi.x = pack_f16x2_sat(f0.x, f0.y); hi.y = pack_f16x2_sat(f1.x, f1.y);
              hi.z = pack_f16x2_sat(f2.x, f2.y); hi.w = pack_f16x2_sat(f3.x, f3.y);
              lo.x = pack_bf16x2(f0.x - f16_lo(hi.x), f0.y - f16_hi(hi.x)); lo.y = pack_bf16x2(f1.x - f16_lo(hi.y), f1.y - f16_hi(hi.y));
              lo.z = pack_bf16x2(f2.x - f16_lo(hi.z), f2.y - f16_hi(hi.z)); lo.w = pack_bf16x2(f3.x - f16_lo(hi.w), f3.y - f16_hi(hi.w));
            }
            const int o = (j ^ swz) << 4;
            *reinterpret_cast<uint4*>(row + o) = hi;
            if (FOLD) *reinterpret_cast<uint4*>(row + SK_A_BYTES + o) = lo;
          }
        }
        fence_async_smem();
        mbar_arrive_local(smem_u32(&a_full[buf]));
        buf += 2;
        if (buf >= SF_NBUF) { buf -= SF_NBUF; ++use; }
      }
      mbar_arrive_local(smem_u32(&halo_free[hb]));
    }
  } else if (warp < 12) {
    const int q = warp & 3, lane = tid & 31;
    float* stage = reinterpret_cast<float*>(bp + SF_OFF_E + (size_t)q * 4096);
    int it = 0;
    for (int tile = blockIdx.x; tile < ntiles; tile += gridDim.x, ++it) {
      const SkTile t = sk_tile(tile, tilesX, tilesY);
      const int ab = it & 1;
      mbar_wait(smem_u32(&acc_full[ab]), (uint32_t)((it >> 1) & 1));
      tc_fence_after();
      const uint32_t tm = tmem_base + ((uint32_t)(q * 32) << 16) + (uint32_t)ab * 128;
#pragma unroll 1
      for (int j = 0; j < 2; ++j) {
        uint32_t u[32], r[32];
        float v[32];
        tmem_ld32(tm + (uint32_t)(j * 32), u);
        if (FOLD) tmem_ld32(tm + (uint32_t)(64 + j * 32), r);
        if (j == 1) {
          tc_fence_before();
          mbar_arrive_local(smem_u32(&acc_empty[ab]));
        }
#pragma unroll
        for (int i = 0; i < 32; ++i) v[i] = FOLD ? fmaf(__uint_as_float(r[i]), 0x1p-11f, __uint_as_float(u[i])) : __uint_as_float(u[i]);
        sk_store_slice(v, stage, lane, q, j, t, OH, OW, bias, out, split_plane);
      }
    }
  } else if (warp == 13) {
    if ((tid & 31) == 0) sk_halo_producer(&tmX, base + SF_OFF_H, halo_full, halo_free, tilesX, tilesY, ntiles, &tmX2, nfirst);
  } else if ((tid & 31) == 0) {
    mbar_expect_tx(smem_u32(&w_bar), SF_BM_BYTES + SF_BC_BYTES);
    bulk_load_1d(b_addr, wtc + SF_IMAGE_OFFSET_FLOATS, SF_BM_BYTES, smem_u32(&w_bar));
    bulk_load_1d(b_addr + SF_BM_BYTES, wtc + SF_IMAGE_OFFSET_FLOATS + SF_BM_BYTES / 4, SF_BC_BYTES, smem_u32(&w_bar));
    mbar_wait(smem_u32(&w_bar), 0);
    int it = 0, buf = 0;
    uint32_t ph = 0;
    for (int tile = blockIdx.x; tile < ntiles; tile += gridDim.x, ++it) {
      const int ab = it & 1;
      mbar_wait(smem_u32(&acc_empty[ab]), (uint32_t)(((it >> 1) & 1) ^ 1));
      tc_fence_after();
      const uint32_t d = tmem_base + (uint32_t)ab * 128;
#pragma unroll
      for (int kt = 0; kt < SF_KSTEPS; ++kt) {
        mbar_wait(smem_u32(&a_full[buf]), ph);
        tc_fence_after();
        const uint32_t a_addr = base + (uint32_t)buf * SF_A_BUF;
        const uint64_t ah = umma_desc_sw128(a_addr), al = umma_desc_sw128(a_addr + SK_A_BYTES);
        const uint64_t bm = umma_desc_sw128(b_addr + (uint32_t)kt * SF_BM_STEP);
        const uint64_t bc = umma_desc_sw128(b_addr + SF_BM_BYTES + (uint32_t)kt * SF_BC_STEP);
        constexpr int NK = 4;
#pragma unroll
        for (int k = 0; k < NK; ++k)
          if (kt < 2 || k < 3) umma_bf16(d, ah + (uint64_t)(2 * k), bm + (uint64_t)(2 * k), FOLD ? SF_IDESC_MAIN : SF_IDESC_ONE, (kt | k) ? 1u : 0u);
        if (FOLD) {
#pragma unroll
          for (int k = 0; k < NK; ++k)
            if (kt < 2 || k < 3) umma_bf16(d, al + (uint64_t)(2 * k), bc + (uint64_t)(2 * k), SF_IDESC_CORR, 1u);
        }
        umma_commit(smem_u32(&a_free[buf]));
        if (++buf == SF_NBUF) { buf = 0; ph ^= 1u; }
      }
      umma_commit(smem_u32(&acc_full[ab]));
    }
  }
  tc_fence_before();
  __syncthreads();
  if (warp == 0) {
    tc_fence_after();
    tmem_dealloc(tmem_base, 256);
  }
}
}

int dh_launch_stem_tc(const float* x, long long xbs, int N, int H, int W, const float* wtc, const float* b, float* out,
                      int x3, cudaStream_t s, long long split_plane_pitch, const float* x_second) {
  const bool split = (x3 & 256) != 0, h16 = (x3 & 512) != 0;
  DH_REQUIRE(!(x3 & ~(255 | 256 | 512)) && !(split && h16), DH_E_VARIANT);
  x3 &= 255;
  DH_REQUIRE(!x_second || x3 == 2 || x3 == 3, DH_E_VARIANT);
  DH_REQUIRE(!split || x3 == 2 || x3 == 3, DH_E_VARIANT);
  DH_REQUIRE(!h16 || x3 == 3, DH_E_VARIANT);
  DH_REQUIRE(x && wtc && b && out, DH_E_NULL);
  DH_REQUIRE(N > 0 && H >= 8 && W >= 8 && H % 2 == 0 && W % 2 == 0, DH_E_SHAPE);
  DH_REQUIRE(dh_aligned16(wtc) && dh_aligned16(b) && dh_aligned16(out), DH_E_ALIGN);
  DH_REQUIRE((reinterpret_cast<uintptr_t>(x) & 3u) == 0, DH_E_ALIGN);
  const int OH = H / 2, OW = W / 2;
  const int tx = dh_cdiv(OW, SK_TW), ty = dh_cdiv(OH, SK_TH);
  const int nimg = x_second ? 2 * N : N;
  const int ntiles = tx * ty * nimg;
  const long long split_plane = h16 ? -1 : split ? (split_plane_pitch ? split_plane_pitch : (long long)nimg * OH * OW * 64) : 0;
  int dev = 0, sms = 148;
  cudaGetDevice(&dev);
  cudaDeviceGetAttribute(&sms, cudaDevAttrMultiProcessorCount, dev);
  dim3 grid((unsigned)(ntiles < sms ? ntiles : sms), 1, 1);
  DH_REQUIRE(W % 4 == 0 && xbs % 4 == 0 && dh_aligned16(x), DH_E_ALIGN);
  CUtensorMap tmX;
  {
    const unsigned long long dims[4] = {(unsigned long long)W, (unsigned long long)H, 3ull, (unsigned long long)N};
    const unsigned long long strides[3] = {(unsigned long long)W * 4, (unsigned long long)H * W * 4, (unsigned long long)xbs * 4};
    const unsigned box[4] = {(unsigned)SK_HCP, (unsigned)SK_HR, 3u, 1u};
    const int rc = dh_encode_tiled_f32(&tmX, x, 4, dims, strides, box, false);
    if (rc) return rc;
  }
  CUtensorMap tmX2 = tmX;
  if (x_second) {
    DH_REQUIRE(dh_aligned16(x_second), DH_E_ALIGN);
    const unsigned long long dims[4] = {(unsigned long long)W, (unsigned long long)H, 3ull, (unsigned long long)N};
    const unsigned long long strides[3] = {(unsigned long long)W * 4, (unsigned long long)H * W * 4, (unsigned long long)xbs * 4};
    const unsigned box[4] = {(unsigned)SK_HCP, (unsigned)SK_HR, 3u, 1u};
    const int rc = dh_encode_tiled_f32(&tmX2, x_second, 4, dims, strides, box, false);
    if (rc) return rc;
  }
  const int nfirst = x_second ? N : (1 << 30);
  if (x3 == 2) {
    cudaError_t e = cudaFuncSetAttribute(stem_f16_kernel<true>, cudaFuncAttributeMaxDynamicSharedMemorySize, (int)SF_SMEM);
    if (e != cudaSuccess) return (int)e;
    return dh_launch(stem_f16_kernel<true>, grid, dim3(SK_THREADS), SF_SMEM, s, tmX, tmX2, nfirst, OH, OW, tx, ty, ntiles, wtc, b, out, split_plane);
  } else if (x3 == 3) {
    cudaError_t e = cudaFuncSetAttribute(stem_f16_kernel<false>, cudaFuncAttributeMaxDynamicSharedMemorySize, (int)SF_SMEM);
    if (e != cudaSuccess) return (int)e;
    return dh_launch(stem_f16_kernel<false>, grid, dim3(SK_THREADS), SF_SMEM, s, tmX, tmX2, nfirst, OH, OW, tx, ty, ntiles, wtc, b, out, split_plane);
  } else if (x3) {
    cudaError_t e = cudaFuncSetAttribute(stem_tc_kernel<true>, cudaFuncAttributeMaxDynamicSharedMemorySize, (int)SkCfg<true>::SMEM);
    if (e != cudaSuccess) return (int)e;
    stem_tc_kernel<true><<<grid, SK_THREADS, SkCfg<true>::SMEM, s>>>(tmX, OH, OW, tx, ty, ntiles, wtc, b, out);
  } else {
    cudaError_t e = cudaFuncSetAttribute(stem_tc_kernel<false>, cudaFuncAttributeMaxDynamicSharedMemorySize, (int)SkCfg<false>::SMEM);
    if (e != cudaSuccess) return (int)e;
    stem_tc_kernel<false><<<grid, SK_THREADS, SkCfg<false>::SMEM, s>>>(tmX, OH, OW, tx, ty, ntiles, wtc, b, out);
  }
  DH_CHECK_LAUNCH();
  return 0;
}
```

### dahitra_b200/csrc/tc_common.cuh

```cuda
#pragma once
#include "common.cuh"
#include <cuda.h>
#include <cstdio>

int dh_encode_tiled_f32(CUtensorMap* out, const void* ptr, int rank, const unsigned long long* dims,
                        const unsigned long long* strides, const unsigned* box, bool swizzle128);
int dh_encode_tiled_f32_sw(CUtensorMap* out, const void* ptr, int rank, const unsigned long long* dims,
                           const unsigned long long* strides, const unsigned* box, int swizzle_bytes);
int dh_encode_tiled_f16_sw(CUtensorMap* out, const void* ptr, int rank, const unsigned long long* dims,
                           const unsigned long long* strides, const unsigned* box, int swizzle_bytes);

namespace dhtc {

__device__ __forceinline__ uint32_t smem_u32(const void* p) { return (uint32_t)__cvta_generic_to_shared(p); }

__device__ __forceinline__ void mbar_init(uint32_t bar, uint32_t count) {
  asm volatile("mbarrier.init.shared::cta.b64 [%0], %1;" ::"r"(bar), "r"(count) : "memory");
}
__device__ __forceinline__ void mbar_fence_init() { asm volatile("fence.mbarrier_init.release.cluster;" ::: "memory"); }
__device__ __forceinline__ void mbar_expect_tx(uint32_t bar, uint32_t bytes) {
  asm volatile("mbarrier.arrive.expect_tx.shared::cta.b64 _, [%0], %1;" ::"r"(bar), "r"(bytes) : "memory");
}
__device__ __forceinline__ void pdl_wait() { asm volatile("griddepcontrol.wait;" ::: "memory"); }
__device__ __forceinline__ void pdl_launch_dependents() { asm volatile("griddepcontrol.launch_dependents;" ::: "memory"); }

__device__ __forceinline__ void mbar_wait(uint32_t bar, uint32_t parity) {
  uint32_t done;
#ifdef DH_MBAR_TIMEOUT
  uint32_t spins = 0;
#endif
  do {
    asm volatile(
        "{\n\t.reg .pred p;\n\t"
        "mbarrier.try_wait.parity.shared::cta.b64 p, [%1], %2, %3;\n\t"
        "selp.u32 %0, 1, 0, p;\n\t}"
        : "=r"(done) : "r"(bar), "r"(parity), "r"(10000u) : "memory");
#ifdef DH_MBAR_TIMEOUT
    if (!done && ++spins > (1u << 19)) {
      printf("[mbar timeout] block %d thread %d bar smem+0x%x parity %u\n", blockIdx.x, threadIdx.x, bar, parity);
      __trap();
    }
#endif
  } while (!done);
}
__device__ __forceinline__ uint32_t cluster_ctarank() { uint32_t r; asm volatile("mov.u32 %0, %%cluster_ctarank;" : "=r"(r)); return r; }
__device__ __forceinline__ void cluster_sync_all() {
  asm volatile("barrier.cluster.arrive.release.aligned;" ::: "memory");
  asm volatile("barrier.cluster.wait.acquire.aligned;" ::: "memory");
}
__device__ __forceinline__ uint32_t mapa_u32(uint32_t smem_addr, uint32_t rank) {
  uint32_t r;
  asm volatile("mapa.shared::cluster.u32 %0, %1, %2;" : "=r"(r) : "r"(smem_addr), "r"(rank));
  return r;
}
__device__ __forceinline__ void mbar_arrive_local(uint32_t bar) {
  asm volatile("mbarrier.arrive.shared::cta.b64 _, [%0];" ::"r"(bar) : "memory");
}
__device__ __forceinline__ void mbar_arrive_cluster(uint32_t cluster_bar) {
  asm volatile("mbarrier.arrive.release.cluster.shared::cluster.b64 _, [%0];" ::"r"(cluster_bar) : "memory");
}
__device__ __forceinline__ void mbar_wait_cluster(uint32_t bar, uint32_t parity) {
  uint32_t done;
#ifdef DH_MBAR_TIMEOUT
  uint32_t spins = 0;
#endif
  do {
    asm volatile(
        "{\n\t.reg .pred p;\n\t"
        "mbarrier.try_wait.parity.acquire.cluster.shared::cta.b64 p, [%1], %2, %3;\n\t"
        "selp.u32 %0, 1, 0, p;\n\t}"
        : "=r"(done) : "r"(bar), "r"(parity), "r"(10000u) : "memory");
#ifdef DH_MBAR_TIMEOUT
    if (!done && ++spins > (1u << 19)) __trap();
#endif
  } while (!done);
}
__device__ __forceinline__ void tma_load_4d_2sm(uint32_t dst, const CUtensorMap* tm, uint32_t cluster_bar, int c0, int c1, int c2, int c3) {
  asm volatile(
      "cp.async.bulk.tensor.4d.cta_group::2.shared::cluster.global.tile.mbarrier::complete_tx::bytes [%0], [%1, {%3, %4, %5, %6}], [%2];"
      ::"r"(dst), "l"(tm), "r"(cluster_bar), "r"(c0), "r"(c1), "r"(c2), "r"(c3) : "memory");
}
__device__ __forceinline__ void tma_load_2d_2sm(uint32_t dst, const CUtensorMap* tm, uint32_t cluster_bar, int c0, int c1) {
  asm volatile(
      "cp.async.bulk.tensor.2d.cta_group::2.shared::cluster.global.tile.mbarrier::complete_tx::bytes [%0], [%1, {%3, %4}], [%2];"
      ::"r"(dst), "l"(tm), "r"(cluster_bar), "r"(c0), "r"(c1) : "memory");
}
__device__ __forceinline__ float tf32_round(float v) {
  return __uint_as_float((__float_as_uint(v) + 0x1000u) & 0xFFFFE000u);
}
__device__ __forceinline__ void tma_load_4d(uint32_t dst, const CUtensorMap* tm, uint32_t bar, int c0, int c1, int c2, int c3) {
  asm volatile(
      "cp.async.bulk.tensor.4d.shared::cluster.global.tile.mbarrier::complete_tx::bytes [%0], [%1, {%3, %4, %5, %6}], [%2];"
      ::"r"(dst), "l"(tm), "r"(bar), "r"(c0), "r"(c1), "r"(c2), "r"(c3) : "memory");
}
__device__ __forceinline__ void tma_load_2d(uint32_t dst, const CUtensorMap* tm, uint32_t bar, int c0, int c1) {
  asm volatile(
      "cp.async.bulk.tensor.2d.shared::cluster.global.tile.mbarrier::complete_tx::bytes [%0], [%1, {%3, %4}], [%2];"
      ::"r"(dst), "l"(tm), "r"(bar), "r"(c0), "r"(c1) : "memory");
}
__device__ __forceinline__ void bulk_load_1d(uint32_t dst, const void* src, uint32_t bytes, uint32_t bar) {
  asm volatile("cp.async.bulk.shared::cluster.global.mbarrier::complete_tx::bytes [%0], [%1], %2, [%3];"
               ::"r"(dst), "l"(src), "r"(bytes), "r"(bar) : "memory");
}
__device__ __forceinline__ void fence_async_smem() { asm volatile("fence.proxy.async.shared::cta;" ::: "memory"); }
__device__ __forceinline__ void tc_fence_before() { asm volatile("tcgen05.fence::before_thread_sync;" ::: "memory"); }
__device__ __forceinline__ void tc_fence_after() { asm volatile("tcgen05.fence::after_thread_sync;" ::: "memory"); }

__device__ __forceinline__ uint64_t umma_desc_sw128(uint32_t smem_addr) {
  return (uint64_t)((smem_addr & 0x3FFFF) >> 4) | ((uint64_t)1 << 16) | ((uint64_t)(1024 >> 4) << 32) |
         ((uint64_t)1 << 46) | ((uint64_t)2 << 61);
}
__host__ __device__ constexpr uint32_t umma_idesc_tf32(int M, int N) {
  return (1u << 4) | (2u << 7) | (2u << 10) | ((uint32_t)(N >> 3) << 17) | ((uint32_t)(M >> 4) << 24);
}
__device__ __forceinline__ void umma_tf32(uint32_t tmem_d, uint64_t adesc, uint64_t bdesc, uint32_t idesc, uint32_t accumulate) {
  asm volatile(
      "{\n\t.reg .pred p;\n\t"
      "setp.ne.b32 p, %4, 0;\n\t"
      "tcgen05.mma.cta_group::1.kind::tf32 [%0], %1, %2, %3, p;\n\t}"
      ::"r"(tmem_d), "l"(adesc), "l"(bdesc), "r"(idesc), "r"(accumulate) : "memory");
}
__device__ __forceinline__ uint64_t umma_desc_sw64(uint32_t smem_addr, uint32_t sbo_bytes) {
  return (uint64_t)((smem_addr & 0x3FFFF) >> 4) | ((uint64_t)1 << 16) | ((uint64_t)(sbo_bytes >> 4) << 32) |
         ((uint64_t)1 << 46) | ((uint64_t)4 << 61);
}
__host__ __device__ constexpr uint32_t umma_idesc_bf16(int M, int N) {
  return (1u << 4) | (1u << 7) | (1u << 10) | ((uint32_t)(N >> 3) << 17) | ((uint32_t)(M >> 4) << 24);
}
__device__ __forceinline__ void umma_bf16(uint32_t tmem_d, uint64_t adesc, uint64_t bdesc, uint32_t idesc, uint32_t accumulate) {
  asm volatile(
      "{\n\t.reg .pred p;\n\t"
      "setp.ne.b32 p, %4, 0;\n\t"
      "tcgen05.mma.cta_group::1.kind::f16 [%0], %1, %2, %3, p;\n\t}"
      ::"r"(tmem_d), "l"(adesc), "l"(bdesc), "r"(idesc), "r"(accumulate) : "memory");
}
__host__ __device__ constexpr uint32_t umma_idesc_f16(int M, int N) {
  return (1u << 4) | ((uint32_t)(N >> 3) << 17) | ((uint32_t)(M >> 4) << 24);
}
__device__ __forceinline__ uint32_t pack_f16x2_sat(float lo, float hi) {
  uint32_t r;
  asm("cvt.rn.satfinite.f16x2.f32 %0, %1, %2;" : "=r"(r) : "f"(hi), "f"(lo));
  return r;
}
__device__ __forceinline__ float f16_lo(uint32_t p) { float f; asm("{ .reg .b16 l, h; mov.b32 {l, h}, %1; cvt.f32.f16 %0, l; }" : "=f"(f) : "r"(p)); return f; }
__device__ __forceinline__ float f16_hi(uint32_t p) { float f; asm("{ .reg .b16 l, h; mov.b32 {l, h}, %1; cvt.f32.f16 %0, h; }" : "=f"(f) : "r"(p)); return f; }
__device__ __forceinline__ uint32_t pack_bf16x2(float lo, float hi) {
  uint32_t r;
  asm("cvt.rn.bf16x2.f32 %0, %1, %2;" : "=r"(r) : "f"(hi), "f"(lo));
  return r;
}
__device__ __forceinline__ void umma_tf32_ts(uint32_t tmem_d, uint32_t tmem_a, uint64_t bdesc, uint32_t idesc, uint32_t accumulate) {
  asm volatile(
      "{\n\t.reg .pred p;\n\t"
      "setp.ne.b32 p, %4, 0;\n\t"
      "tcgen05.mma.cta_group::1.kind::tf32 [%0], [%1], %2, %3, p;\n\t}"
      ::"r"(tmem_d), "r"(tmem_a), "l"(bdesc), "r"(idesc), "r"(accumulate) : "memory");
}
__device__ __forceinline__ void umma_tf32_2sm(uint32_t tmem_d, uint64_t adesc, uint64_t bdesc, uint32_t idesc, uint32_t accumulate) {
  asm volatile(
      "{\n\t.reg .pred p;\n\t"
      "setp.ne.b32 p, %4, 0;\n\t"
      "tcgen05.mma.cta_group::2.kind::tf32 [%0], %1, %2, %3, p;\n\t}"
      ::"r"(tmem_d), "l"(adesc), "l"(bdesc), "r"(idesc), "r"(accumulate) : "memory");
}
__device__ __forceinline__ void umma_bf16_2sm(uint32_t tmem_d, uint64_t adesc, uint64_t bdesc, uint32_t idesc, uint32_t accumulate) {
  asm volatile(
      "{\n\t.reg .pred p;\n\t"
      "setp.ne.b32 p, %4, 0;\n\t"
      "tcgen05.mma.cta_group::2.kind::f16 [%0], %1, %2, %3, p;\n\t}"
      ::"r"(tmem_d), "l"(adesc), "l"(bdesc), "r"(idesc), "r"(accumulate) : "memory");
}
__device__ __forceinline__ void umma_commit_2sm(uint32_t bar) {
  asm volatile("tcgen05.commit.cta_group::2.mbarrier::arrive::one.shared::cluster.multicast::cluster.b64 [%0], %1;"
               ::"r"(bar), "h"((uint16_t)3) : "memory");
}
__device__ __forceinline__ void tmem_alloc_2sm(uint32_t slot_smem_addr, uint32_t ncols) {
  asm volatile("tcgen05.alloc.cta_group::2.sync.aligned.shared::cta.b32 [%0], %1;" ::"r"(slot_smem_addr), "r"(ncols) : "memory");
  asm volatile("tcgen05.relinquish_alloc_permit.cta_group::2.sync.aligned;" ::: "memory");
}
__device__ __forceinline__ void tmem_dealloc_2sm(uint32_t taddr, uint32_t ncols) {
  asm volatile("tcgen05.dealloc.cta_group::2.sync.aligned.b32 %0, %1;" ::"r"(taddr), "r"(ncols) : "memory");
}
__device__ __forceinline__ void umma_commit(uint32_t bar) {
  asm volatile("tcgen05.commit.cta_group::1.mbarrier::arrive::one.shared::cluster.b64 [%0];" ::"r"(bar) : "memory");
}
__device__ __forceinline__ void tmem_alloc(uint32_t slot_smem_addr, uint32_t ncols) {
  asm volatile("tcgen05.alloc.cta_group::1.sync.aligned.shared::cta.b32 [%0], %1;" ::"r"(slot_smem_addr), "r"(ncols) : "memory");
  asm volatile("tcgen05.relinquish_alloc_permit.cta_group::1.sync.aligned;" ::: "memory");
}
__device__ __forceinline__ void tmem_dealloc(uint32_t taddr, uint32_t ncols) {
  asm volatile("tcgen05.dealloc.cta_group::1.sync.aligned.b32 %0, %1;" ::"r"(taddr), "r"(ncols) : "memory");
}
__device__ __forceinline__ void tmem_ld32(uint32_t taddr, uint32_t (&v)[32]) {
  asm volatile(
      "tcgen05.ld.sync.aligned.32x32b.x32.b32 "
      "{%0, %1, %2, %3, %4, %5, %6, %7, %8, %9, %10, %11, %12, %13, %14, %15, "
      "%16, %17, %18, %19, %20, %21, %22, %23, %24, %25, %26, %27, %28, %29, %30, %31}, [%32];"
      : "=r"(v[0]), "=r"(v[1]), "=r"(v[2]), "=r"(v[3]), "=r"(v[4]), "=r"(v[5]), "=r"(v[6]), "=r"(v[7]),
        "=r"(v[8]), "=r"(v[9]), "=r"(v[10]), "=r"(v[11]), "=r"(v[12]), "=r"(v[13]), "=r"(v[14]), "=r"(v[15]),
        "=r"(v[16]), "=r"(v[17]), "=r"(v[18]), "=r"(v[19]), "=r"(v[20]), "=r"(v[21]), "=r"(v[22]), "=r"(v[23]),
        "=r"(v[24]), "=r"(v[25]), "=r"(v[26]), "=r"(v[27]), "=r"(v[28]), "=r"(v[29]), "=r"(v[30]), "=r"(v[31])
      : "r"(taddr) : "memory");
  asm volatile("tcgen05.wait::ld.sync.aligned;" ::: "memory");
}
__device__ __forceinline__ void tmem_ld16(uint32_t taddr, uint32_t (&v)[16]) {
  asm volatile(
      "tcgen05.ld.sync.aligned.32x32b.x16.b32 "
      "{%0, %1, %2, %3, %4, %5, %6, %7, %8, %9, %10, %11, %12, %13, %14, %15}, [%16];"
      : "=r"(v[0]), "=r"(v[1]), "=r"(v[2]), "=r"(v[3]), "=r"(v[4]), "=r"(v[5]), "=r"(v[6]), "=r"(v[7]),
        "=r"(v[8]), "=r"(v[9]), "=r"(v[10]), "=r"(v[11]), "=r"(v[12]), "=r"(v[13]), "=r"(v[14]), "=r"(v[15])
      : "r"(taddr) : "memory");
  asm volatile("tcgen05.wait::ld.sync.aligned;" ::: "memory");
}
__device__ __forceinline__ void tmem_st32(uint32_t taddr, const uint32_t (&v)[32]) {
  asm volatile(
      "tcgen05.st.sync.aligned.32x32b.x32.b32 [%0], "
      "{%1, %2, %3, %4, %5, %6, %7, %8, %9, %10, %11, %12, %13, %14, %15, %16, "
      "%17, %18, %19, %20, %21, %22, %23, %24, %25, %26, %27, %28, %29, %30, %31, %32};"
      ::"r"(taddr), "r"(v[0]), "r"(v[1]), "r"(v[2]), "r"(v[3]), "r"(v[4]), "r"(v[5]), "r"(v[6]), "r"(v[7]),
        "r"(v[8]), "r"(v[9]), "r"(v[10]), "r"(v[11]), "r"(v[12]), "r"(v[13]), "r"(v[14]), "r"(v[15]),
        "r"(v[16]), "r"(v[17]), "r"(v[18]), "r"(v[19]), "r"(v[20]), "r"(v[21]), "r"(v[22]), "r"(v[23]),
        "r"(v[24]), "r"(v[25]), "r"(v[26]), "r"(v[27]), "r"(v[28]), "r"(v[29]), "r"(v[30]), "r"(v[31])
      : "memory");
  asm volatile("tcgen05.wait::st.sync.aligned;" ::: "memory");
}

__device__ __forceinline__ unsigned long long f2_pack(float2 a) { unsigned long long r; asm("mov.b64 %0, {%1, %2};" : "=l"(r) : "f"(a.x), "f"(a.y)); return r; }
__device__ __forceinline__ float2 f2_unpack(unsigned long long r) { float2 d; asm("mov.b64 {%0, %1}, %2;" : "=f"(d.x), "=f"(d.y) : "l"(r)); return d; }
__device__ __forceinline__ float2 ffma2(float2 a, float2 b, float2 c) {
  unsigned long long d; asm("fma.rn.f32x2 %0, %1, %2, %3;" : "=l"(d) : "l"(f2_pack(a)), "l"(f2_pack(b)), "l"(f2_pack(c))); return f2_unpack(d);
}
__device__ __forceinline__ float2 fadd2(float2 a, float2 b) { unsigned long long d; asm("add.rn.f32x2 %0, %1, %2;" : "=l"(d) : "l"(f2_pack(a)), "l"(f2_pack(b))); return f2_unpack(d); }
__device__ __forceinline__ float2 fsub2(float2 a, float2 b) { unsigned long long d; asm("sub.rn.f32x2 %0, %1, %2;" : "=l"(d) : "l"(f2_pack(a)), "l"(f2_pack(b))); return f2_unpack(d); }
__device__ __forceinline__ float2 fmul2(float2 a, float2 b) { unsigned long long d; asm("mul.rn.f32x2 %0, %1, %2;" : "=l"(d) : "l"(f2_pack(a)), "l"(f2_pack(b))); return f2_unpack(d); }
__device__ __forceinline__ float2 f2_bcast(float s) { return make_float2(s, s); }

__host__ __device__ __forceinline__ int sw128_idx(int r, int k) { return r * 32 + ((((k >> 2) ^ (r & 7)) << 2) | (k & 3)); }

}
```

### include/dahitra_b200.h

```cpp
#ifndef DAHITRA_B200_H
#define DAHITRA_B200_H

#include <stddef.h>
#include <stdint.h>

#ifdef __cplusplus
extern "C" {
#endif

#define DAHITRA_ABI_VERSION 2

#define DH_E_NULL      (-1)
#define DH_E_SHAPE     (-2)
#define DH_E_ALIGN     (-3)
#define DH_E_WORKSPACE (-4)
#define DH_E_VARIANT   (-5)
#define DH_E_WEIGHTS   (-6)

#define DH_VARIANT_LEVIR 0
#define DH_VARIANT_XBD   1

#define DH_FLAG_NONE        0
#define DH_FLAG_CONV_TC     1
#define DH_FLAG_TC_3XTF32   2
#define DH_FLAG_TC_STRIDE2  4
#define DH_FLAG_DEC_TC      8
#define DH_FLAG_STEM_TC     16
#define DH_FLAG_DEC_TC_X3   32
#define DH_FLAG_CONV_TC_V1  64
#define DH_FLAG_CONV_TC_2CTA 128
#define DH_FLAG_SERIAL      256
#define DH_FLAG_TC_X3_BF16  512
#define DH_FLAG_TC_BF16     1024
#define DH_FLAG_TC_MAIN_F16 2048
#define DH_FLAG_TC_FOLD     4096
#define DH_FLAG_EARLY_HEAD  8192
#define DH_FLAG_ACT_SPLIT   16384
#define DH_FLAG_PDL         32768
#define DH_FLAG_ACT_H16     65536
#define DH_FLAGS_TF32X3     (DH_FLAG_CONV_TC | DH_FLAG_TC_3XTF32 | DH_FLAG_TC_X3_BF16 | DH_FLAG_TC_MAIN_F16 | DH_FLAG_TC_FOLD | DH_FLAG_TC_STRIDE2 | \
                             DH_FLAG_STEM_TC | DH_FLAG_DEC_TC | DH_FLAG_DEC_TC_X3 | DH_FLAG_ACT_SPLIT | DH_FLAG_PDL)
#define DH_FLAGS_TF32       (DH_FLAG_CONV_TC | DH_FLAG_TC_STRIDE2 | DH_FLAG_STEM_TC | DH_FLAG_DEC_TC | DH_FLAG_DEC_TC_X3)
#define DH_FLAGS_F16        (DH_FLAGS_TF32 | DH_FLAG_TC_MAIN_F16)
#define DH_FLAGS_BF16       (DH_FLAGS_TF32 | DH_FLAG_TC_BF16)
#define DH_FLAGS_H16        (DH_FLAGS_F16 | DH_FLAG_ACT_H16 | DH_FLAG_PDL)

enum dh_weight_slot {
  DH_W_STEM_W = 0, DH_W_STEM_B,
  DH_W_L1_0_C1_W, DH_W_L1_0_C1_B, DH_W_L1_0_C2_W, DH_W_L1_0_C2_B,
  DH_W_L1_1_C1_W, DH_W_L1_1_C1_B, DH_W_L1_1_C2_W, DH_W_L1_1_C2_B,
  DH_W_L2_0_C1_W, DH_W_L2_0_C1_B, DH_W_L2_0_C2_W, DH_W_L2_0_C2_B, DH_W_L2_0_DS_W, DH_W_L2_0_DS_B,
  DH_W_L2_1_C1_W, DH_W_L2_1_C1_B, DH_W_L2_1_C2_W, DH_W_L2_1_C2_B,
  DH_W_L3_0_C1_W, DH_W_L3_0_C1_B, DH_W_L3_0_C2_W, DH_W_L3_0_C2_B, DH_W_L3_0_DS_W, DH_W_L3_0_DS_B,
  DH_W_L3_1_C1_W, DH_W_L3_1_C1_B, DH_W_L3_1_C2_W, DH_W_L3_1_C2_B,
  DH_W_LV5_SQ, DH_W_LV5_TOK, DH_W_LV5_ENC, DH_W_LV5_DEC, DH_W_LV5_POS, DH_W_LV5_DECODE,
  DH_W_LV4_SQ, DH_W_LV4_TOK, DH_W_LV4_ENC, DH_W_LV4_DEC, DH_W_LV4_POS, DH_W_LV4_DECODE,
  DH_W_LV3_SQ, DH_W_LV3_TOK, DH_W_LV3_ENC, DH_W_LV3_DEC, DH_W_LV3_POS, DH_W_LV3_DECODE,
  DH_W_CL4_W, DH_W_CL4_B, DH_W_CL3_W, DH_W_CL3_B, DH_W_CL2_W, DH_W_CL2_B,
  DH_W_CL20A_W, DH_W_CL20A_B,
  DH_W_CL20B_W, DH_W_CL20B_B,
  DH_W_CLS_W, DH_W_CLS_B,
  DH_W_L1_0_C1_WT, DH_W_L1_0_C2_WT, DH_W_L1_1_C1_WT, DH_W_L1_1_C2_WT,
  DH_W_L2_0_C2_WT, DH_W_L2_1_C1_WT, DH_W_L2_1_C2_WT,
  DH_W_L3_0_C1_WT, DH_W_L3_0_C2_WT, DH_W_L3_0_DS_WT, DH_W_L3_1_C1_WT, DH_W_L3_1_C2_WT,
  DH_W_LV5_DECODE_WT, DH_W_LV4_DECODE_WT, DH_W_LV3_DECODE_WT,
  DH_W_CL20A_WT, DH_W_CL20B_WT,
  DH_W_L2_0_C1_WT, DH_W_L2_0_DS_WT,
  DH_W_CL4_PSWT, DH_W_CL4_PSB, DH_W_CL3_PSWT, DH_W_CL3_PSB, DH_W_CL2_PSWT, DH_W_CL2_PSB,
  DH_W_LV5_DECTC, DH_W_LV4_DECTC, DH_W_LV3_DECTC,
  DH_W_STEM_WTC,
  DH_W_LV5_SQ_WT, DH_W_LV4_SQ_WT, DH_W_LV3_SQ_WT,
  DH_W_COUNT
};

#define DH_ENC_FLOATS(H)       (8*32 + 64 + 2*(H)*1024 + 32 + 64 + 1024 + 32 + 1024 + 32)
#define DH_DEC_LAYER_FLOATS(H) (64 + 2*(H)*1024 + 32 + 1024 + 32 + 1024 + 32)

int         dahitra_version(void);
const char* dahitra_error_string(int code);
const char* dahitra_weight_slot_name(int slot);

#define DH_DTYPE_F32 0
#define DH_DTYPE_F64 1
typedef struct dh_tensor { const char* name; const void* data; int dtype; int ndim; long long shape[4]; } dh_tensor;
long long dahitra_prepare_weights(const dh_tensor* tensors, int n_tensors, int variant, int output_nc,
                                  float* out, long long out_floats, long long* slot_offsets);

size_t dahitra_workspace_bytes(int variant, int B, int H, int W, int output_nc, int flags);

int dahitra_forward(const void* const* weights, int n_weights,
                    const float* x1, const float* x2, long long x_batch_stride,
                    float* logits, unsigned char* argmax_u8,
                    void* workspace, size_t workspace_bytes,
                    int variant, int B, int H, int W, int output_nc, int flags, void* stream);

int dahitra_forward_profiled(const void* const* weights, int n_weights,
                             const float* x1, const float* x2, long long x_batch_stride,
                             float* logits, unsigned char* argmax_u8,
                             void* workspace, size_t workspace_bytes,
                             int variant, int B, int H, int W, int output_nc, int flags, void* stream,
                             int cap, float* ms, double* flops, double* bytes, const char** names);


int dahitra_conv2d(const float* in0, const float* in1, int C0, int C1, int N, int inH, int inW, int up,
                   int KH, int KW, int stride, int pad, int Cout,
                   const float* w, const float* wt, const float* bias, const float* res, int relu,
                   float* out, int flags, void* stream);

int dahitra_conv2d_up2_tc(const float* in, int N, int inH, int inW, const float* pswt, const float* psb,
                          int relu, float* out, int flags, void* stream);

int dahitra_stem(const float* x, long long x_batch_stride, int N, int H, int W,
                 const float* w, const float* bias, float* out, void* stream);

int dahitra_stem_tc(const float* x, long long x_batch_stride, int N, int H, int W,
                    const float* wtc, const float* bias, float* out, int x3, void* stream);

int dahitra_maxpool3x3s2(const float* in, int N, int H, int W, int C, float* out, void* stream);

int dahitra_squeeze_tokens(const float* feat, int N, int npix, int Cin, const float* w_sq, const float* w_tok,
                           float* xs, float* partials, void* stream);

int dahitra_token_encoder(const float* partials, int B, int nchunk, const float* enc_pack, int heads, int add_pos,
                          float* mem, void* stream);

#define DH_TAB_FLOATS(H) (32*4*(H) + 4*(H) + 4*(H)*32 + 32)
int dahitra_decoder_tables(const float* mem, int B, int first_call, int ncalls, const float* dec_pack, int heads, int depth,
                           float* tables, void* stream);

int dahitra_pixel_decoder(const float* x, const float* pos, const float* tables, const float* dec_pack,
                          int nimg, int h, int w, int heads, int depth, const float* skip, int skip_up, float* out,
                          void* stream);

#define DH_TABTC_FLOATS        (1024 + 1024 + 32 + 2048)
#define DH_DECTC_LAYER_FLOATS  (1024 + 1024 + 32 + 32 + 32 + 2048)
int dahitra_decoder_tables_tc(const float* mem, int B, int first_call, int ncalls, const float* dec_pack, int heads,
                              int depth, float* tables, void* stream);
int dahitra_pixel_decoder_tc(const float* x, const float* pos, const float* tables, const float* dectc_pack,
                             int nimg, int h, int w, int heads, int depth, const float* skip, int skip_up, int x3,
                             float* out, void* stream);

int dahitra_split_pack(const float* in, long long n, void* out_split, void* stream);
int dahitra_split_unpack(const void* in_split, long long n, float* out, void* stream);
int dahitra_maxpool3x3s2_split(const void* in_split, int N, int H, int W, int C, void* out_split, void* stream);
int dahitra_maxpool3x3s2_h16(const void* in_h16, int N, int H, int W, int C, void* out_h16, void* stream);
int dahitra_conv2d_split(const void* in0, const void* in1, int C0, int C1, long long in0_plane, long long in1_plane,
                         int N, int inH, int inW, int K, int stride, int Cout, const float* wt, const float* bias,
                         const void* res, int res_split, int relu, void* out, int out_split, int mode,
                         const float* w_tok, float* partials, void* stream);

int dahitra_classifier(const float* in, int N, int H, int W, int nc, const float* w, const float* bias,
                       float* logits, unsigned char* argmax_u8, void* stream);
int dahitra_classifier_h16(const void* in_h16, int N, int H, int W, int nc, const float* w, const float* bias,
                           float* logits, unsigned char* argmax_u8, void* stream);

#define DH_TRAIN_TAB_FLOATS(H) (65*4*(H) + 96 + 2048)
int dahitra_pixel_decoder_train_blocks(int npix);
int dahitra_pixel_decoder_train_fwd(const float* x, const float* tables, float* xs, float* out, int nimg, int npix,
                                    int heads, int depth, int pixel_major, void* stream);
int dahitra_pixel_decoder_train_bwd(const float* dout, const float* xs, const float* tables, float* dx,
                                    float* dtables_partial, int nimg, int npix, int heads, int depth, int pixel_major,
                                    void* stream);

int dahitra_tokenizer_train_chunks(int npix);
int dahitra_tokenizer_train_fwd(const float* x, const float* w_tok, float* partials, float* tokens, float* stats,
                                int nimg, int npix, int pixel_major, void* stream);
int dahitra_tokenizer_train_bwd(const float* x, const float* w_tok, const float* tokens, const float* stats,
                                const float* dtokens, float* dx, float* dw_partial, int nimg, int npix, int pixel_major,
                                void* stream);


int dahitra_confusion_matrix(const unsigned char* pred, const unsigned char* gt, long long n, int nc,
                             long long* cm, void* stream);

int dahitra_prepare_input_u8(const unsigned char* hwc, int N, int H, int W, int kind, int tile, float* nchw, void* stream);

#ifdef __cplusplus
}
#endif
#endif
```

Baseline: 17080.

## Rewrite f16 stem as space-to-depth UMMA kernel with fused 3x3s2 maxpool

```diff
diff --git a/dahitra_b200/_lib.py b/dahitra_b200/_lib.py
--- a/dahitra_b200/_lib.py
+++ b/dahitra_b200/_lib.py
@@ -130,6 +130,7 @@
     "dahitra_conv2d_up2_tc": (_I, [_P, _I, _I, _I, _P, _P, _I, _P, _I, _P]),
     "dahitra_stem": (_I, [_P, _LL, _I, _I, _I, _P, _P, _P, _P]),
     "dahitra_stem_tc": (_I, [_P, _LL, _I, _I, _I, _P, _P, _P, _I, _P]),
+    "dahitra_stem_pool_tc": (_I, [_P, _LL, _I, _I, _I, _P, _P, _P, _P, _I, _P]),
     "dahitra_maxpool3x3s2": (_I, [_P, _I, _I, _I, _I, _P, _P]),
     "dahitra_squeeze_tokens": (_I, [_P, _I, _I, _I, _P, _P, _P, _P, _P]),
     "dahitra_token_encoder": (_I, [_P, _I, _I, _P, _I, _I, _P, _P]),
diff --git a/dahitra_b200/csrc/common.cuh b/dahitra_b200/csrc/common.cuh
--- a/dahitra_b200/csrc/common.cuh
+++ b/dahitra_b200/csrc/common.cuh
@@ -97,7 +97,8 @@
 int dh_launch_conv_tc2(const ConvArgs& a, int xm, int cg, cudaStream_t s);
 int dh_launch_stem(const float* x, long long xbs, int N, int H, int W, const float* w, const float* b, float* out, cudaStream_t s);
 int dh_launch_stem_tc(const float* x, long long xbs, int N, int H, int W, const float* wtc, const float* b, float* out, int x3,
-                      cudaStream_t s, long long split_plane_pitch = 0, const float* x_second = nullptr);
+                      cudaStream_t s, long long split_plane_pitch = 0, const float* x_second = nullptr, float* pooled = nullptr,
+                      long long pool_plane_pitch = 0);
 int dh_launch_maxpool(const float* in, int N, int H, int W, int C, float* out, cudaStream_t s);
 int dh_launch_classifier(const float* in, int N, int H, int W, int nc, const float* w, const float* b,
                          float* logits, unsigned char* amax, cudaStream_t s);
diff --git a/dahitra_b200/csrc/forward.cu b/dahitra_b200/csrc/forward.cu
--- a/dahitra_b200/csrc/forward.cu
+++ b/dahitra_b200/csrc/forward.cu
@@ -163,6 +163,11 @@
 extern "C" int dahitra_stem_tc(const float* x, long long xbs, int N, int H, int W, const float* wtc, const float* bias,
                                float* out, int x3, void* stream) {
   return dh_launch_stem_tc(x, xbs, N, H, W, wtc, bias, out, x3, (cudaStream_t)stream);
+}
+extern "C" int dahitra_stem_pool_tc(const float* x, long long xbs, int N, int H, int W, const float* wtc, const float* bias,
+                                    float* out, void* pooled_out, int x3, void* stream) {
+  DH_REQUIRE(pooled_out, DH_E_NULL);
+  return dh_launch_stem_tc(x, xbs, N, H, W, wtc, bias, out, x3, (cudaStream_t)stream, 0, nullptr, static_cast<float*>(pooled_out));
 }
 extern "C" int dahitra_maxpool3x3s2(const float* in, int N, int H, int W, int C, float* out, void* stream) {
   return dh_launch_maxpool(in, N, H, W, C, out, (cudaStream_t)stream);
@@ -346,13 +351,12 @@
   const double stem_fl = 2.0 * B * h2 * w2 * 64 * 147;
   const double stem_by = one ? B * (4.0 * 3 * H * W + 2.0 * h2 * w2 * 64) : 4.0 * B * ((double)3 * H * W + (double)h2 * w2 * 64);
   const int stem_mode = one ? 3 | 512 : ((flags & DH_FLAG_TC_3XTF32) ? 2 : 3) | 256;
-  DH_STEP("stem", 2.0 * stem_fl, 2.0 * stem_by,
-          dh_launch_stem_tc(x1, x_batch_stride, B, H, W, Wt(DH_W_STEM_WTC), Wt(DH_W_STEM_B), F2, stem_mode, s, f2_plane, x2));
   float* P2 = ws + p.p2;
+  DH_STEP("stem_pool", 2.0 * stem_fl, 2.0 * stem_by + eb * N2 * 64 * (double)h4 * w4,
+          dh_launch_stem_tc(x1, x_batch_stride, B, H, W, Wt(DH_W_STEM_WTC), Wt(DH_W_STEM_B), F2, stem_mode, s, f2_plane, x2, P2));
   auto maxpool = [&](const float* in, int hh, int ww, int C, float* out) {
     return one ? dh_launch_maxpool_h16(in, N2, hh, ww, C, out, s) : dh_launch_maxpool_split(in, N2, hh, ww, C, out, s);
   };
-  DH_STEP("maxpool_2", 0.0, eb * N2 * 64 * ((double)h2 * w2 + (double)h4 * w4), maxpool(F2, h2, w2, 64, P2));
   float *T4a = ws + p.t4a, *T4b = ws + p.t4b, *F4 = ws + p.f4;
   DH_CONV3("layer1.0.conv1", P2, nullptr, 64, 0, 0, N2, h4, w4, 3, 1, 64, DH_W_L1_0_C1_WT, DH_W_L1_0_C1_B, nullptr, 0, 1, T4a, 1, 0);
   DH_CONV3("layer1.0.conv2", T4a, nullptr, 64, 0, 0, N2, h4, w4, 3, 1, 64, DH_W_L1_0_C2_WT, DH_W_L1_0_C2_B, P2, 1, 1, T4b, 1, 0);
diff --git a/dahitra_b200/csrc/stem_tc.cu b/dahitra_b200/csrc/stem_tc.cu
--- a/dahitra_b200/csrc/stem_tc.cu
+++ b/dahitra_b200/csrc/stem_tc.cu
@@ -50,25 +50,25 @@
   }
 }
 
-__device__ __forceinline__ void sk_store_slice(const float (&v)[32], float* stage, int lane, int q, int j, const SkTile& t,
-                                               int OH, int OW, const float* __restrict__ bias, float* __restrict__ out,
+__device__ __forceinline__ void sk_store_slice(const float (&v)[32], float* stage, int lane, int q, int j, int n, int oy0, int ox0,
+                                               int tw, int OH, int OW, const float* __restrict__ bias, float* __restrict__ out,
                                                long long split_plane = 0) {
   const int c4 = lane & 3, r4 = lane >> 2;
 #pragma unroll
   for (int k4 = 0; k4 < 8; ++k4)
     *reinterpret_cast<float4*>(stage + lane * 32 + ((k4 ^ (lane & 7)) << 2)) = make_float4(v[k4 * 4], v[k4 * 4 + 1], v[k4 * 4 + 2], v[k4 * 4 + 3]);
   __syncwarp();
-  const float4 b0 = ldg4(bias + j * 32 + c4 * 8), b1 = ldg4(bias + j * 32 + c4 * 8 + 4);
+  const float4 b0 = bias ? ldg4(bias + j * 32 + c4 * 8) : float4{}, b1 = bias ? ldg4(bias + j * 32 + c4 * 8 + 4) : float4{};
 #pragma unroll
   for (int g = 0; g < 4; ++g) {
     const int r = g * 8 + r4, mm = q * 32 + r;
-    const int oy = t.oy0 + mm / SK_TW, ox = t.ox0 + mm % SK_TW;
+    const int oy = oy0 + mm / tw, ox = ox0 + mm % tw;
     const float4 o0 = *reinterpret_cast<const float4*>(stage + r * 32 + (((2 * c4) ^ (r & 7)) << 2));
     const float4 o1 = *reinterpret_cast<const float4*>(stage + r * 32 + (((2 * c4 + 1) ^ (r & 7)) << 2));
     if (oy < OH && ox < OW) {
-      const float4 r0 = make_float4(fmaxf(o0.x + b0.x, 0.f), fmaxf(o0.y + b0.y, 0.f), fmaxf(o0.z + b0.z, 0.f), fmaxf(o0.w + b0.w, 0.f));
-      const float4 r1 = make_float4(fmaxf(o1.x + b1.x, 0.f), fmaxf(o1.y + b1.y, 0.f), fmaxf(o1.z + b1.z, 0.f), fmaxf(o1.w + b1.w, 0.f));
-      const size_t off = ((size_t)(t.n * OH + oy) * OW + ox) * 64 + j * 32 + c4 * 8;
+      const float4 r0 = !bias ? o0 : make_float4(fmaxf(o0.x + b0.x, 0.f), fmaxf(o0.y + b0.y, 0.f), fmaxf(o0.z + b0.z, 0.f), fmaxf(o0.w + b0.w, 0.f));
+      const float4 r1 = !bias ? o1 : make_float4(fmaxf(o1.x + b1.x, 0.f), fmaxf(o1.y + b1.y, 0.f), fmaxf(o1.z + b1.z, 0.f), fmaxf(o1.w + b1.w, 0.f));
+      const size_t off = ((size_t)(n * OH + oy) * OW + ox) * 64 + j * 32 + c4 * 8;
       if (split_plane < 0) {
         uint4 hi;
         hi.x = pack_f16x2_sat(r0.x, r0.y); hi.y = pack_f16x2_sat(r0.z, r0.w); hi.z = pack_f16x2_sat(r1.x, r1.y); hi.w = pack_f16x2_sat(r1.z, r1.w);
@@ -184,7 +184,7 @@
         }
 #pragma unroll
         for (int i = 0; i < 32; ++i) v[i] = __uint_as_float(u[i]);
-        sk_store_slice(v, stage, lane, q, j, t, OH, OW, bias, out);
+        sk_store_slice(v, stage, lane, q, j, t.n, t.oy0, t.ox0, SK_TW, OH, OW, bias, out);
       }
     }
   } else if (warp == 13) {
@@ -230,215 +230,394 @@
     tmem_dealloc(tmem_base, 128);
   }
 }
-constexpr int SF_KSTEPS = 3;
-constexpr int SF_NBUF = 3;
-constexpr uint32_t SF_A_BUF = 2 * SK_A_BYTES;
-constexpr uint32_t SF_BM_STEP = 128 * 128;
-constexpr uint32_t SF_BC_STEP = 64 * 128;
-constexpr uint32_t SF_BM_BYTES = SF_KSTEPS * SF_BM_STEP, SF_BC_BYTES = SF_KSTEPS * SF_BC_STEP;
-constexpr uint32_t SF_OFF_B = SF_NBUF * SF_A_BUF;
-constexpr uint32_t SF_OFF_H = SF_OFF_B + SF_BM_BYTES + SF_BC_BYTES;
-constexpr uint32_t SF_OFF_E = SF_OFF_H + 2 * SK_HALO_STRIDE;
-constexpr uint32_t SF_SMEM = SF_OFF_E + 4 * 4096 + 1024;
+constexpr int S2_TW = 128;
+constexpr int S2_XW = S2_TW + 3;
+constexpr uint32_t S2_PLANE = 136 * 16;
+constexpr int S2_RAWC = 132;
+constexpr uint32_t S2_RAW_HALF = 3200;
+constexpr uint32_t S2_RAW = 2 * S2_RAW_HALF;
+constexpr uint32_t S2_RAW_TX = 2 * 3 * 2 * S2_RAWC * 4;
+constexpr int S2_NS = 6, S2_NR = 4;
+constexpr int S2_RMAX = 32;
+constexpr int S2_THREADS = 12 * 32;
+constexpr uint32_t SF_BM_BYTES = 3 * 128 * 128, SF_BC_BYTES = 3 * 64 * 128;
+constexpr size_t SF_IMAGE_OFFSET_FLOATS = 2 * (SK_B_BYTES / 4);
 constexpr uint32_t SF_IDESC_MAIN = umma_idesc_f16(128, 128), SF_IDESC_CORR = umma_idesc_bf16(128, 64), SF_IDESC_ONE = umma_idesc_f16(128, 64);
-constexpr size_t SF_IMAGE_OFFSET_FLOATS = 2 * (SK_B_BYTES / 4);
+
+template <bool FOLD> struct S2Cfg {
+  static constexpr uint32_t NBM = FOLD ? 128 : 64;
+  static constexpr uint32_t BM_TAP = NBM * 32, BC_TAP = FOLD ? 64 * 32 : 0;
+  static constexpr uint32_t OFF_BC = 16 * BM_TAP;
+  static constexpr uint32_t OFF_S = OFF_BC + 16 * BC_TAP;
+  static constexpr uint32_t SLOT = (FOLD ? 4 : 2) * S2_PLANE;
+  static constexpr uint32_t OFF_R = OFF_S + S2_NS * SLOT;
+  static constexpr uint32_t OFF_E = OFF_R + S2_NR * S2_RAW;
+  static constexpr uint32_t OFF_X = OFF_E + 8 * 4096;
+  static constexpr uint32_t OFF_D = OFF_X + 2 * 2 * 4 * 32 * 4;
+  static constexpr uint32_t OFF_B = OFF_D + 2 * (S2_RMAX / 2) * 64 * 4;
+  static constexpr uint32_t SMEM = OFF_B + 64 * 4 + 1024;
+  static constexpr uint32_t STAGE = FOLD ? SF_BM_BYTES + SF_BC_BYTES : SF_BM_BYTES;
+  static_assert(STAGE <= OFF_E - OFF_S, "filter staging overlaps the epilogue buffers");
+  static_assert(OFF_R % 128 == 0, "TMA destinations need 128-byte alignment");
+};
+
+struct S2Unit { int n, y0, ys, ye; };
+__device__ __forceinline__ S2Unit s2_unit(int u, int nbands, int R, int OH, bool pool) {
+  S2Unit w;
+  w.n = u / nbands;
+  w.y0 = (u % nbands) * R;
+  w.ye = min(w.y0 + R, OH);
+  w.ys = pool && w.y0 > 0 ? w.y0 - 1 : w.y0;
+  return w;
+}
+__device__ __forceinline__ void bar_sync_epilogue() { asm volatile("bar.sync 1, 256;" ::: "memory"); }
+__device__ __forceinline__ void bar_sync_half(int j) { asm volatile("bar.sync %0, 128;" ::"r"(2 + j) : "memory"); }
 
 template <bool FOLD>
-__global__ void __launch_bounds__(SK_THREADS, 1)
-stem_f16_kernel(const __grid_constant__ CUtensorMap tmX, const __grid_constant__ CUtensorMap tmX2, int nfirst, int OH, int OW, int tilesX,
-                int tilesY, int ntiles, const float* __restrict__ wtc, const float* __restrict__ bias, float* __restrict__ out,
-                long long split_plane) {
+__global__ void __launch_bounds__(S2_THREADS, 1)
+stem_s2d_kernel(const __grid_constant__ CUtensorMap tmX, const __grid_constant__ CUtensorMap tmX2, int nfirst, int OH, int OW, int ctiles,
+                int nbands, int R, int nunits, const float* __restrict__ wtc, const float* __restrict__ bias, float* __restrict__ out,
+                long long split_plane, float* __restrict__ pooled, long long pool_plane) {
+  using Cfg = S2Cfg<FOLD>;
   extern __shared__ uint8_t sk_raw[];
-  __shared__ __align__(8) uint64_t w_bar, a_full[SF_NBUF], a_free[SF_NBUF], acc_full[2], acc_empty[2], halo_full[2], halo_free[2];
+  __shared__ __align__(8) uint64_t w_bar, raw_full[S2_NR], raw_free[S2_NR], s2_full[S2_NS], s2_free[S2_NS], acc_full[2], acc_empty[2];
   __shared__ uint32_t tmem_slot;
   const int tid = threadIdx.x, warp = tid >> 5;
   const uint32_t base = (smem_u32(sk_raw) + 1023u) & ~1023u;
   uint8_t* bp = sk_raw + (base - smem_u32(sk_raw));
-  const uint32_t b_addr = base + SF_OFF_B;
+  const bool pool = pooled != nullptr;
 
   if (tid == 0) {
     mbar_init(smem_u32(&w_bar), 1);
-    for (int i = 0; i < SF_NBUF; ++i) {
-      mbar_init(smem_u32(&a_full[i]), 128);
-      mbar_init(smem_u32(&a_free[i]), 1);
+    for (int i = 0; i < S2_NR; ++i) {
+      mbar_init(smem_u32(&raw_full[i]), 1);
+      mbar_init(smem_u32(&raw_free[i]), 64);
+    }
+    for (int i = 0; i < S2_NS; ++i) {
+      mbar_init(smem_u32(&s2_full[i]), 64);
+      mbar_init(smem_u32(&s2_free[i]), 1);
     }
     for (int i = 0; i < 2; ++i) {
       mbar_init(smem_u32(&acc_full[i]), 1);
-      mbar_init(smem_u32(&acc_empty[i]), 128);
-      mbar_init(smem_u32(&halo_full[i]), 1);
-      mbar_init(smem_u32(&halo_free[i]), 256);
+      mbar_init(smem_u32(&acc_empty[i]), 256);
     }
     mbar_fence_init();
   }
-  if (warp == 0) tmem_alloc(smem_u32(&tmem_slot), 256);
+  if (warp == 0) tmem_alloc(smem_u32(&tmem_slot), 512);
   tc_fence_before();
   __syncthreads();
   tc_fence_after();
   const uint32_t tmem_base = tmem_slot;
+  if (tid == 0) {
+    mbar_expect_tx(smem_u32(&w_bar), Cfg::STAGE);
+    bulk_load_1d(base + Cfg::OFF_S, wtc + SF_IMAGE_OFFSET_FLOATS, SF_BM_BYTES, smem_u32(&w_bar));
+    if (FOLD) bulk_load_1d(base + Cfg::OFF_S + SF_BM_BYTES, wtc + SF_IMAGE_OFFSET_FLOATS + SF_BM_BYTES / 4, SF_BC_BYTES, smem_u32(&w_bar));
+  }
+  mbar_wait(smem_u32(&w_bar), 0);
+  {
+    const uint16_t* m16 = reinterpret_cast<const uint16_t*>(bp + Cfg::OFF_S);
+    const uint16_t* c16 = m16 + SF_BM_BYTES / 2;
+    constexpr int MAIN_ROWS = 16 * 2 * Cfg::NBM, ROWS = MAIN_ROWS + (FOLD ? 16 * 2 * 64 : 0);
+    for (int i = tid; i < ROWS; i += S2_THREADS) {
+      const bool corr = i >= MAIN_ROWS;
+      const int nrows = corr ? 64 : Cfg::NBM, rr = corr ? i - MAIN_ROWS : i;
+      const int tap = rr / (2 * nrows), plane = (rr / nrows) & 1, n = rr % nrows;
+      const uint16_t* src = corr ? c16 : m16;
+      const int tile_halves = (corr ? 64 : 128) * 64;
+      uint16_t v[8];
+#pragma unroll
+      for (int c = 0; c < 8; ++c) {
+        const int k16 = plane * 8 + c, ci = k16 >> 2;
+        const int r = 2 * (tap >> 2) + ((k16 >> 1) & 1) - 1, s = 2 * (tap & 3) + (k16 & 1) - 1;
+        v[c] = 0;
+        if (k16 < 12 && r >= 0 && s >= 0) {
+          const int K = (ci * 7 + r) * 8 + 1 + s, kk = K & 63;
+          v[c] = src[(K >> 6) * tile_halves + n * 64 + ((((kk >> 3) ^ (n & 7)) << 3) | (kk & 7))];
+        }
+      }
+      const uint32_t dst = corr ? Cfg::OFF_BC + tap * Cfg::BC_TAP + plane * 64 * 16 : tap * Cfg::BM_TAP + plane * Cfg::NBM * 16;
+      *reinterpret_cast<uint4*>(bp + dst + n * 16) = make_uint4(v[0] | (uint32_t)v[1] << 16, v[2] | (uint32_t)v[3] << 16,
+                                                               v[4] | (uint32_t)v[5] << 16, v[6] | (uint32_t)v[7] << 16);
+    }
+  }
+  fence_async_smem();
+  __syncthreads();
   dh_pdl_wait();
   dh_pdl_launch_dependents();
 
   if (warp < 8) {
-    const int wg = warp >> 2, t = tid & 127;
-    const int py = t / SK_TW, px = t % SK_TW;
-    const int pbase = (2 * py) * SK_HCP + 2 * px;
-    const int swz = t & 7;
-    int it = 0, c = wg, buf = wg, use = 0;
-    for (int tile = blockIdx.x; tile < ntiles; tile += gridDim.x, ++it) {
-      const int hb = it & 1;
-      mbar_wait(smem_u32(&halo_full[hb]), (uint32_t)((it >> 1) & 1));
-      const float* halo = reinterpret_cast<const float*>(bp + SF_OFF_H + (size_t)hb * SK_HALO_STRIDE) + pbase;
-#pragma unroll 1
-      for (; c < SF_KSTEPS * (it + 1); c += 2) {
-        const int kt = c - SF_KSTEPS * it;
-        if (use >= 1) mbar_wait(smem_u32(&a_free[buf]), (uint32_t)((use - 1) & 1));
-        uint8_t* row = bp + (size_t)buf * SF_A_BUF + t * 128;
-        const int ng = kt == 2 ? 6 : 8;
-#pragma unroll
-        for (int j = 0; j < 8; ++j) {
-          if (j < ng) {
-            const int g = kt * 8 + j;
-            uint4 hi = make_uint4(0u, 0u, 0u, 0u), lo = hi;
-            if (g < SK_GROUPS) {
-              const float2* src = reinterpret_cast<const float2*>(halo + (g / 7) * SK_PLANE + (g % 7) * SK_HCP);
-              const float2 f0 = src[0], f1 = src[1], f2 = src[2], f3 = src[3];
-              hi.x = pack_f16x2_sat(f0.x, f0.y); hi.y = pack_f16x2_sat(f1.x, f1.y);
-              hi.z = pack_f16x2_sat(f2.x, f2.y); hi.w = pack_f16x2_sat(f3.x, f3.y);
-              lo.x = pack_bf16x2(f0.x - f16_lo(hi.x), f0.y - f16_hi(hi.x)); lo.y = pack_bf16x2(f1.x - f16_lo(hi.y), f1.y - f16_hi(hi.y));
-              lo.z = pack_bf16x2(f2.x - f16_lo(hi.z), f2.y - f16_hi(hi.z)); lo.w = pack_bf16x2(f3.x - f16_lo(hi.w), f3.y - f16_hi(hi.w));
+    const int q = warp & 3, j = warp >> 2, lane = tid & 31;
+    float* stage = reinterpret_cast<float*>(bp + Cfg::OFF_E + (size_t)warp * 4096);
+    float* exch = reinterpret_cast<float*>(bp + Cfg::OFF_X);
+    float* edge = reinterpret_cast<float*>(bp + Cfg::OFF_D);
+    float* sbias = reinterpret_cast<float*>(bp + Cfg::OFF_B);
+    if (tid < 64) sbias[tid] = bias[tid];
+    bar_sync_epilogue();
+    const int PH = OH >> 1, PW = OW >> 1;
+    int go = 0, e = 0;
+    for (int u = blockIdx.x; u < nunits; u += gridDim.x) {
+      const S2Unit w = s2_unit(u, nbands, R, OH, pool);
+      for (int ct = 0; ct < ctiles; ++ct) {
+        const int x0 = ct * S2_TW, x = x0 + q * 32 + lane;
+        for (int y = w.ys; y < w.ye; ++y, ++go) {
+          const int ab = go & 1;
+          mbar_wait(smem_u32(&acc_full[ab]), (uint32_t)((go >> 1) & 1));
+          tc_fence_after();
+          const uint32_t tm = tmem_base + ((uint32_t)(q * 32) << 16) + (uint32_t)ab * 128;
+          const bool emit = pool && (y & 1) && y > w.ys;
+          const int prow = (y - 1 - w.y0) >> 1;
+          {
+            uint32_t ua[32];
+            float f[32];
+            tmem_ld32(tm + (uint32_t)(j * 32), ua);
+            if (FOLD) {
+#pragma unroll
+              for (int h = 0; h < 2; ++h) {
+                uint32_t ur[16];
+                tmem_ld16(tm + (uint32_t)(64 + j * 32 + h * 16), ur);
+#pragma unroll
+                for (int i = 0; i < 16; ++i)
+                  ua[h * 16 + i] = __float_as_uint(fmaf(__uint_as_float(ur[i]), 0x1p-11f, __uint_as_float(ua[h * 16 + i])));
+              }
             }
-            const int o = (j ^ swz) << 4;
-            *reinterpret_cast<uint4*>(row + o) = hi;
-            if (FOLD) *reinterpret_cast<uint4*>(row + SK_A_BYTES + o) = lo;
+            tc_fence_before();
+            mbar_arrive_local(smem_u32(&acc_empty[ab]));
+#pragma unroll
+            for (int i = 0; i < 32; ++i) f[i] = fmaxf(__uint_as_float(ua[i]) + sbias[j * 32 + i], 0.f);
+            if (y >= w.y0) sk_store_slice(f, stage, lane, q, j, w.n, y, x0, S2_TW, OH, OW, nullptr, out, split_plane);
+            if (!pool) continue;
+            const uint32_t tst = tmem_base + ((uint32_t)(q * 32) << 16) + 256u + (uint32_t)(j * 32);
+            uint32_t sv[32];
+            if (y == w.ys) {
+#pragma unroll
+              for (int i = 0; i < 32; ++i) sv[i] = __float_as_uint(f[i]);
+            } else {
+              tmem_ld32(tst, sv);
+#pragma unroll
+              for (int i = 0; i < 32; ++i) {
+                const float v = f[i], m = fmaxf(__uint_as_float(sv[i]), v);
+                if (y & 1) { f[i] = m; sv[i] = __float_as_uint(v); }
+                else sv[i] = __float_as_uint(m);
+              }
+            }
+            tmem_st32(tst, sv);
+            if (!emit) continue;
+            float* ex = exch + ((e & 1) * 2 + j) * 128;
+            float* ed = edge + (size_t)((ct & 1) * (S2_RMAX / 2) + prow) * 64 + j * 32;
+            if (lane == 31) {
+#pragma unroll
+              for (int i = 0; i < 32; ++i) {
+                ex[q * 32 + i] = f[i];
+                if (q == 3) ed[i] = f[i];
+              }
+            }
+            bar_sync_half(j);
+            const float* lp = q ? ex + (q - 1) * 32
+                                : ct ? edge + (size_t)(((ct - 1) & 1) * (S2_RMAX / 2) + prow) * 64 + j * 32 : nullptr;
+            const int py = (y - 1) >> 1;
+            const size_t po = ((size_t)(w.n * PH + py) * PW + (x >> 1)) * 64 + j * 32;
+#pragma unroll
+            for (int k = 0; k < 4; ++k) {
+              float o[8];
+#pragma unroll
+              for (int c = 0; c < 8; ++c) {
+                const int i = 8 * k + c;
+                float l = __shfl_up_sync(0xffffffffu, f[i], 1);
+                const float rt = __shfl_down_sync(0xffffffffu, f[i], 1);
+                if (lane == 0) l = lp ? lp[i] : f[i];
+                o[c] = fmaxf(fmaxf(l, f[i]), rt);
+              }
+              if (!(lane & 1) && x < OW) {
+                uint4 hi;
+                hi.x = pack_f16x2_sat(o[0], o[1]); hi.y = pack_f16x2_sat(o[2], o[3]); hi.z = pack_f16x2_sat(o[4], o[5]); hi.w = pack_f16x2_sat(o[6], o[7]);
+                if (split_plane < 0) {
+                  *reinterpret_cast<uint4*>(reinterpret_cast<uint16_t*>(pooled) + po + 8 * k) = hi;
+                } else if (split_plane) {
+                  uint4 lo;
+                  lo.x = pack_f16x2_sat((o[0] - f16_lo(hi.x)) * 2048.f, (o[1] - f16_hi(hi.x)) * 2048.f);
+                  lo.y = pack_f16x2_sat((o[2] - f16_lo(hi.y)) * 2048.f, (o[3] - f16_hi(hi.y)) * 2048.f);
+                  lo.z = pack_f16x2_sat((o[4] - f16_lo(hi.z)) * 2048.f, (o[5] - f16_hi(hi.z)) * 2048.f);
+                  lo.w = pack_f16x2_sat((o[6] - f16_lo(hi.w)) * 2048.f, (o[7] - f16_hi(hi.w)) * 2048.f);
+                  uint16_t* p16 = reinterpret_cast<uint16_t*>(pooled);
+                  *reinterpret_cast<uint4*>(p16 + po + 8 * k) = hi;
+                  *reinterpret_cast<uint4*>(p16 + po + 8 * k + (size_t)pool_plane) = lo;
+                } else {
+                  st4(pooled + po + 8 * k, make_float4(o[0], o[1], o[2], o[3]));
+                  st4(pooled + po + 8 * k + 4, make_float4(o[4], o[5], o[6], o[7]));
+                }
+              }
+            }
+            ++e;
           }
         }
-        fence_async_smem();
-        mbar_arrive_local(smem_u32(&a_full[buf]));
-        buf += 2;
-        if (buf >= SF_NBUF) { buf -= SF_NBUF; ++use; }
-      }
-      mbar_arrive_local(smem_u32(&halo_free[hb]));
-    }
-  } else if (warp < 12) {
-    const int q = warp & 3, lane = tid & 31;
-    float* stage = reinterpret_cast<float*>(bp + SF_OFF_E + (size_t)q * 4096);
-    int it = 0;
-    for (int tile = blockIdx.x; tile < ntiles; tile += gridDim.x, ++it) {
-      const SkTile t = sk_tile(tile, tilesX, tilesY);
-      const int ab = it & 1;
-      mbar_wait(smem_u32(&acc_full[ab]), (uint32_t)((it >> 1) & 1));
-      tc_fence_after();
-      const uint32_t tm = tmem_base + ((uint32_t)(q * 32) << 16) + (uint32_t)ab * 128;
-#pragma unroll 1
-      for (int j = 0; j < 2; ++j) {
-        uint32_t u[32], r[32];
-        float v[32];
-        tmem_ld32(tm + (uint32_t)(j * 32), u);
-        if (FOLD) tmem_ld32(tm + (uint32_t)(64 + j * 32), r);
-        if (j == 1) {
-          tc_fence_before();
-          mbar_arrive_local(smem_u32(&acc_empty[ab]));
-        }
-#pragma unroll
-        for (int i = 0; i < 32; ++i) v[i] = FOLD ? fmaf(__uint_as_float(r[i]), 0x1p-11f, __uint_as_float(u[i])) : __uint_as_float(u[i]);
-        sk_store_slice(v, stage, lane, q, j, t, OH, OW, bias, out, split_plane);
-      }
-    }
-  } else if (warp == 13) {
-    if ((tid & 31) == 0) sk_halo_producer(&tmX, base + SF_OFF_H, halo_full, halo_free, tilesX, tilesY, ntiles, &tmX2, nfirst);
+      }
+    }
+  } else if (warp < 10) {
+    const int t = tid - 256;
+    int g = 0;
+    for (int u = blockIdx.x; u < nunits; u += gridDim.x) {
+      const S2Unit w = s2_unit(u, nbands, R, OH, pool);
+      for (int ct = 0; ct < ctiles; ++ct) {
+        for (int Y = w.ys - 2; Y <= w.ye; ++Y, ++g) {
+          const int r = g % S2_NR, s = g % S2_NS;
+          mbar_wait(smem_u32(&raw_full[r]), (uint32_t)((g / S2_NR) & 1));
+          if (g >= S2_NS) mbar_wait(smem_u32(&s2_free[s]), (uint32_t)(((g / S2_NS) - 1) & 1));
+          const float* rw = reinterpret_cast<const float*>(bp + Cfg::OFF_R + (size_t)r * S2_RAW);
+          uint8_t* sl = bp + Cfg::OFF_S + (size_t)s * Cfg::SLOT;
+          for (int i = t; i < S2_XW; i += 64) {
+            const int h = i >= S2_RAWC / 2;
+            const float* p = rw + h * (S2_RAW_HALF / 4) + 2 * i - h * S2_RAWC;
+            float2 a[6];
+#pragma unroll
+            for (int k = 0; k < 6; ++k) a[k] = *reinterpret_cast<const float2*>(p + k * S2_RAWC);
+            uint32_t hv[6];
+#pragma unroll
+            for (int k = 0; k < 6; ++k) hv[k] = pack_f16x2_sat(a[k].x, a[k].y);
+            *reinterpret_cast<uint4*>(sl + i * 16) = make_uint4(hv[0], hv[1], hv[2], hv[3]);
+            *reinterpret_cast<uint4*>(sl + S2_PLANE + i * 16) = make_uint4(hv[4], hv[5], 0u, 0u);
+            if (FOLD) {
+              uint32_t lv[6];
+#pragma unroll
+              for (int k = 0; k < 6; ++k) lv[k] = pack_bf16x2(a[k].x - f16_lo(hv[k]), a[k].y - f16_hi(hv[k]));
+              *reinterpret_cast<uint4*>(sl + 2 * S2_PLANE + i * 16) = make_uint4(lv[0], lv[1], lv[2], lv[3]);
+              *reinterpret_cast<uint4*>(sl + 3 * S2_PLANE + i * 16) = make_uint4(lv[4], lv[5], 0u, 0u);
+            }
+          }
+          mbar_arrive_local(smem_u32(&raw_free[r]));
+          fence_async_smem();
+          mbar_arrive_local(smem_u32(&s2_full[s]));
+        }
+      }
+    }
+  } else if (warp == 11) {
+    if ((tid & 31) == 0) {
+      int g = 0;
+      for (int u = blockIdx.x; u < nunits; u += gridDim.x) {
+        const S2Unit w = s2_unit(u, nbands, R, OH, pool);
+        const bool second = w.n >= nfirst;
+        const CUtensorMap* tm = second ? &tmX2 : &tmX;
+        const int ni = second ? w.n - nfirst : w.n;
+        for (int ct = 0; ct < ctiles; ++ct) {
+          for (int Y = w.ys - 2; Y <= w.ye; ++Y, ++g) {
+            const int r = g % S2_NR;
+            if (g >= S2_NR) mbar_wait(smem_u32(&raw_free[r]), (uint32_t)(((g / S2_NR) - 1) & 1));
+            const uint32_t bar = smem_u32(&raw_full[r]), dst = base + Cfg::OFF_R + (uint32_t)r * S2_RAW;
+            mbar_expect_tx(bar, S2_RAW_TX);
+            tma_load_4d(dst, tm, bar, 2 * ct * S2_TW - 4, 2 * Y, 0, ni);
+            tma_load_4d(dst + S2_RAW_HALF, tm, bar, 2 * ct * S2_TW - 4 + S2_RAWC, 2 * Y, 0, ni);
+          }
+        }
+      }
+    }
   } else if ((tid & 31) == 0) {
-    mbar_expect_tx(smem_u32(&w_bar), SF_BM_BYTES + SF_BC_BYTES);
-    bulk_load_1d(b_addr, wtc + SF_IMAGE_OFFSET_FLOATS, SF_BM_BYTES, smem_u32(&w_bar));
-    bulk_load_1d(b_addr + SF_BM_BYTES, wtc + SF_IMAGE_OFFSET_FLOATS + SF_BM_BYTES / 4, SF_BC_BYTES, smem_u32(&w_bar));
-    mbar_wait(smem_u32(&w_bar), 0);
-    int it = 0, buf = 0;
-    uint32_t ph = 0;
-    for (int tile = blockIdx.x; tile < ntiles; tile += gridDim.x, ++it) {
-      const int ab = it & 1;
-      mbar_wait(smem_u32(&acc_empty[ab]), (uint32_t)(((it >> 1) & 1) ^ 1));
-      tc_fence_after();
-      const uint32_t d = tmem_base + (uint32_t)ab * 128;
-#pragma unroll
-      for (int kt = 0; kt < SF_KSTEPS; ++kt) {
-        mbar_wait(smem_u32(&a_full[buf]), ph);
-        tc_fence_after();
-        const uint32_t a_addr = base + (uint32_t)buf * SF_A_BUF;
-        const uint64_t ah = umma_desc_sw128(a_addr), al = umma_desc_sw128(a_addr + SK_A_BYTES);
-        const uint64_t bm = umma_desc_sw128(b_addr + (uint32_t)kt * SF_BM_STEP);
-        const uint64_t bc = umma_desc_sw128(b_addr + SF_BM_BYTES + (uint32_t)kt * SF_BC_STEP);
-        constexpr int NK = 4;
-#pragma unroll
-        for (int k = 0; k < NK; ++k)
-          if (kt < 2 || k < 3) umma_bf16(d, ah + (uint64_t)(2 * k), bm + (uint64_t)(2 * k), FOLD ? SF_IDESC_MAIN : SF_IDESC_ONE, (kt | k) ? 1u : 0u);
-        if (FOLD) {
-#pragma unroll
-          for (int k = 0; k < NK; ++k)
-            if (kt < 2 || k < 3) umma_bf16(d, al + (uint64_t)(2 * k), bc + (uint64_t)(2 * k), SF_IDESC_CORR, 1u);
-        }
-        umma_commit(smem_u32(&a_free[buf]));
-        if (++buf == SF_NBUF) { buf = 0; ph ^= 1u; }
-      }
-      umma_commit(smem_u32(&acc_full[ab]));
+    int g = 0, gw = 0, go = 0;
+    for (int u = blockIdx.x; u < nunits; u += gridDim.x) {
+      const S2Unit w = s2_unit(u, nbands, R, OH, pool);
+      const int nr = w.ye - w.ys;
+      for (int ct = 0; ct < ctiles; ++ct) {
+        for (int jr = 0; jr < nr; ++jr, ++go) {
+          const int ab = go & 1;
+          mbar_wait(smem_u32(&acc_empty[ab]), (uint32_t)(((go >> 1) & 1) ^ 1));
+          for (; gw <= g + jr + 3; ++gw) mbar_wait(smem_u32(&s2_full[gw % S2_NS]), (uint32_t)((gw / S2_NS) & 1));
+          tc_fence_after();
+          const uint32_t d = tmem_base + (uint32_t)ab * 128;
+#pragma unroll
+          for (int dy = 0; dy < 4; ++dy) {
+            const uint32_t sa = base + Cfg::OFF_S + (uint32_t)((g + jr + dy) % S2_NS) * Cfg::SLOT;
+#pragma unroll
+            for (int dx = 0; dx < 4; ++dx) {
+              const int tap = dy * 4 + dx;
+              const uint64_t ah = umma_desc_nosw(sa + dx * 16, S2_PLANE, 128);
+              const uint64_t bm = umma_desc_nosw(base + tap * Cfg::BM_TAP, Cfg::NBM * 16, 128);
+              umma_bf16(d, ah, bm, FOLD ? SF_IDESC_MAIN : SF_IDESC_ONE, tap ? 1u : 0u);
+              if (FOLD) {
+                const uint64_t al = umma_desc_nosw(sa + 2 * S2_PLANE + dx * 16, S2_PLANE, 128);
+                const uint64_t bc = umma_desc_nosw(base + Cfg::OFF_BC + tap * Cfg::BC_TAP, 64 * 16, 128);
+                umma_bf16(d, al, bc, SF_IDESC_CORR, 1u);
+              }
+            }
+          }
+          umma_commit(smem_u32(&acc_full[ab]));
+          umma_commit(smem_u32(&s2_free[(g + jr) % S2_NS]));
+        }
+        for (int k = nr; k < nr + 3; ++k) umma_commit(smem_u32(&s2_free[(g + k) % S2_NS]));
+        g += nr + 3;
+      }
     }
   }
   tc_fence_before();
   __syncthreads();
   if (warp == 0) {
     tc_fence_after();
-    tmem_dealloc(tmem_base, 256);
+    tmem_dealloc(tmem_base, 512);
   }
 }
 }
 
 int dh_launch_stem_tc(const float* x, long long xbs, int N, int H, int W, const float* wtc, const float* b, float* out,
-                      int x3, cudaStream_t s, long long split_plane_pitch, const float* x_second) {
+                      int x3, cudaStream_t s, long long split_plane_pitch, const float* x_second, float* pooled,
+                      long long pool_plane_pitch) {
   const bool split = (x3 & 256) != 0, h16 = (x3 & 512) != 0;
   DH_REQUIRE(!(x3 & ~(255 | 256 | 512)) && !(split && h16), DH_E_VARIANT);
   x3 &= 255;
   DH_REQUIRE(!x_second || x3 == 2 || x3 == 3, DH_E_VARIANT);
   DH_REQUIRE(!split || x3 == 2 || x3 == 3, DH_E_VARIANT);
   DH_REQUIRE(!h16 || x3 == 3, DH_E_VARIANT);
+  DH_REQUIRE(!pooled || x3 == 2 || x3 == 3, DH_E_VARIANT);
   DH_REQUIRE(x && wtc && b && out, DH_E_NULL);
   DH_REQUIRE(N > 0 && H >= 8 && W >= 8 && H % 2 == 0 && W % 2 == 0, DH_E_SHAPE);
-  DH_REQUIRE(dh_aligned16(wtc) && dh_aligned16(b) && dh_aligned16(out), DH_E_ALIGN);
+  DH_REQUIRE(!pooled || (H % 4 == 0 && W % 4 == 0), DH_E_SHAPE);
+  DH_REQUIRE(dh_aligned16(wtc) && dh_aligned16(b) && dh_aligned16(out) && (!pooled || dh_aligned16(pooled)), DH_E_ALIGN);
   DH_REQUIRE((reinterpret_cast<uintptr_t>(x) & 3u) == 0, DH_E_ALIGN);
   const int OH = H / 2, OW = W / 2;
-  const int tx = dh_cdiv(OW, SK_TW), ty = dh_cdiv(OH, SK_TH);
   const int nimg = x_second ? 2 * N : N;
-  const int ntiles = tx * ty * nimg;
   const long long split_plane = h16 ? -1 : split ? (split_plane_pitch ? split_plane_pitch : (long long)nimg * OH * OW * 64) : 0;
+  const long long pool_plane = pool_plane_pitch ? pool_plane_pitch : (long long)nimg * (OH / 2) * (OW / 2) * 64;
   int dev = 0, sms = 148;
   cudaGetDevice(&dev);
   cudaDeviceGetAttribute(&sms, cudaDevAttrMultiProcessorCount, dev);
-  dim3 grid((unsigned)(ntiles < sms ? ntiles : sms), 1, 1);
   DH_REQUIRE(W % 4 == 0 && xbs % 4 == 0 && dh_aligned16(x), DH_E_ALIGN);
-  CUtensorMap tmX;
-  {
-    const unsigned long long dims[4] = {(unsigned long long)W, (unsigned long long)H, 3ull, (unsigned long long)N};
-    const unsigned long long strides[3] = {(unsigned long long)W * 4, (unsigned long long)H * W * 4, (unsigned long long)xbs * 4};
-    const unsigned box[4] = {(unsigned)SK_HCP, (unsigned)SK_HR, 3u, 1u};
-    const int rc = dh_encode_tiled_f32(&tmX, x, 4, dims, strides, box, false);
-    if (rc) return rc;
-  }
-  CUtensorMap tmX2 = tmX;
+  const bool s2d = x3 >= 2;
+  const unsigned box[4] = {s2d ? (unsigned)S2_RAWC : (unsigned)SK_HCP, s2d ? 2u : (unsigned)SK_HR, 3u, 1u};
+  const unsigned long long dims[4] = {(unsigned long long)W, (unsigned long long)H, 3ull, (unsigned long long)N};
+  const unsigned long long strides[3] = {(unsigned long long)W * 4, (unsigned long long)H * W * 4, (unsigned long long)xbs * 4};
+  CUtensorMap tmX, tmX2;
+  int rc = dh_encode_tiled_f32(&tmX, x, 4, dims, strides, box, false);
+  if (rc) return rc;
+  tmX2 = tmX;
   if (x_second) {
     DH_REQUIRE(dh_aligned16(x_second), DH_E_ALIGN);
-    const unsigned long long dims[4] = {(unsigned long long)W, (unsigned long long)H, 3ull, (unsigned long long)N};
-    const unsigned long long strides[3] = {(unsigned long long)W * 4, (unsigned long long)H * W * 4, (unsigned long long)xbs * 4};
-    const unsigned box[4] = {(unsigned)SK_HCP, (unsigned)SK_HR, 3u, 1u};
-    const int rc = dh_encode_tiled_f32(&tmX2, x_second, 4, dims, strides, box, false);
+    rc = dh_encode_tiled_f32(&tmX2, x_second, 4, dims, strides, box, false);
     if (rc) return rc;
   }
-  const int nfirst = x_second ? N : (1 << 30);
-  if (x3 == 2) {
-    cudaError_t e = cudaFuncSetAttribute(stem_f16_kernel<true>, cudaFuncAttributeMaxDynamicSharedMemorySize, (int)SF_SMEM);
+  if (s2d) {
+    int R = S2_RMAX;
+    long long best = -1;
+    for (int r = 8; r <= S2_RMAX; r += 2) {
+      const long long units = (long long)nimg * dh_cdiv(OH, r);
+      const long long cost = (units + sms - 1) / sms * (r + (pooled ? 1 : 0) + (pooled ? 0 : 3));
+      if (best < 0 || cost < best) { best = cost; R = r; }
+    }
+    const int nbands = dh_cdiv(OH, R), ctiles = dh_cdiv(OW, S2_TW);
+    const long long nunits = (long long)nimg * nbands;
+    DH_REQUIRE(nunits < (1ll << 31), DH_E_SHAPE);
+    const dim3 grid((unsigned)(nunits < sms ? nunits : sms));
+    const int nfirst = x_second ? N : (1 << 30);
+    if (x3 == 2) {
+      cudaError_t e = cudaFuncSetAttribute(stem_s2d_kernel<true>, cudaFuncAttributeMaxDynamicSharedMemorySize, (int)S2Cfg<true>::SMEM);
+      if (e != cudaSuccess) return (int)e;
+      return dh_launch(stem_s2d_kernel<true>, grid, dim3(S2_THREADS), S2Cfg<true>::SMEM, s, tmX, tmX2, nfirst, OH, OW, ctiles, nbands, R,
+                       (int)nunits, wtc, b, out, split_plane, pooled, pool_plane);
+    }
+    cudaError_t e = cudaFuncSetAttribute(stem_s2d_kernel<false>, cudaFuncAttributeMaxDynamicSharedMemorySize, (int)S2Cfg<false>::SMEM);
     if (e != cudaSuccess) return (int)e;
-    return dh_launch(stem_f16_kernel<true>, grid, dim3(SK_THREADS), SF_SMEM, s, tmX, tmX2, nfirst, OH, OW, tx, ty, ntiles, wtc, b, out, split_plane);
-  } else if (x3 == 3) {
-    cudaError_t e = cudaFuncSetAttribute(stem_f16_kernel<false>, cudaFuncAttributeMaxDynamicSharedMemorySize, (int)SF_SMEM);
-    if (e != cudaSuccess) return (int)e;
-    return dh_launch(stem_f16_kernel<false>, grid, dim3(SK_THREADS), SF_SMEM, s, tmX, tmX2, nfirst, OH, OW, tx, ty, ntiles, wtc, b, out, split_plane);
-  } else if (x3) {
+    return dh_launch(stem_s2d_kernel<false>, grid, dim3(S2_THREADS), S2Cfg<false>::SMEM, s, tmX, tmX2, nfirst, OH, OW, ctiles, nbands, R,
+                     (int)nunits, wtc, b, out, split_plane, pooled, pool_plane);
+  }
+  const int tx = dh_cdiv(OW, SK_TW), ty = dh_cdiv(OH, SK_TH);
+  const int ntiles = tx * ty * nimg;
+  dim3 grid((unsigned)(ntiles < sms ? ntiles : sms), 1, 1);
+  if (x3) {
     cudaError_t e = cudaFuncSetAttribute(stem_tc_kernel<true>, cudaFuncAttributeMaxDynamicSharedMemorySize, (int)SkCfg<true>::SMEM);
     if (e != cudaSuccess) return (int)e;
     stem_tc_kernel<true><<<grid, SK_THREADS, SkCfg<true>::SMEM, s>>>(tmX, OH, OW, tx, ty, ntiles, wtc, b, out);
diff --git a/dahitra_b200/csrc/tc_common.cuh b/dahitra_b200/csrc/tc_common.cuh
--- a/dahitra_b200/csrc/tc_common.cuh
+++ b/dahitra_b200/csrc/tc_common.cuh
@@ -123,6 +123,10 @@
 __device__ __forceinline__ uint64_t umma_desc_sw64(uint32_t smem_addr, uint32_t sbo_bytes) {
   return (uint64_t)((smem_addr & 0x3FFFF) >> 4) | ((uint64_t)1 << 16) | ((uint64_t)(sbo_bytes >> 4) << 32) |
          ((uint64_t)1 << 46) | ((uint64_t)4 << 61);
+}
+__device__ __forceinline__ uint64_t umma_desc_nosw(uint32_t smem_addr, uint32_t k_stride, uint32_t m_stride) {
+  return (uint64_t)((smem_addr & 0x3FFFF) >> 4) | ((uint64_t)(k_stride >> 4) << 16) | ((uint64_t)(m_stride >> 4) << 32) |
+         ((uint64_t)1 << 46);
 }
 __host__ __device__ constexpr uint32_t umma_idesc_bf16(int M, int N) {
   return (1u << 4) | (1u << 7) | (1u << 10) | ((uint32_t)(N >> 3) << 17) | ((uint32_t)(M >> 4) << 24);
diff --git a/include/dahitra_b200.h b/include/dahitra_b200.h
--- a/include/dahitra_b200.h
+++ b/include/dahitra_b200.h
@@ -115,6 +115,8 @@
 
 int dahitra_stem_tc(const float* x, long long x_batch_stride, int N, int H, int W,
                     const float* wtc, const float* bias, float* out, int x3, void* stream);
+int dahitra_stem_pool_tc(const float* x, long long x_batch_stride, int N, int H, int W,
+                         const float* wtc, const float* bias, float* out, void* pooled_out, int x3, void* stream);
 
 int dahitra_maxpool3x3s2(const float* in, int N, int H, int W, int C, float* out, void* stream);
 
```

Measured after the change: 17730 (median of 6 runs). +3.8%, better.
